# francescobrigante/Audio-Style-Transfer

Hardware: AMD Instinct MI355X
Metric: audio-seconds/sec/node (train step, 4s@22.05kHz pairs) (higher is better)
Workload: dtype bf16; 1 GPU; configs[1]: batch=8 4 s clips per GPU (S=2, x=(B,S,2,287,597)), full train2 step: STFT + CQT front-end from resident waveforms, encoders+decoder+discriminator, all losses, D and G phases, grad clip, Adam; global_batch=8, parallelism=dp1, hip_graph=True, dp_semantics=per-rank BN and batch-coupled losses

## Files before the change

audio-style-transfer_amd/ast_amd/_lib.py:

```python
from __future__ import annotations

import ctypes as C
import os

import torch

_HERE = os.path.dirname(os.path.abspath(__file__))
LIB_PATH = os.environ.get("AST_HIP_LIB") or os.path.join(_HERE, "libast_hip.so")

F32, BF16 = 0, 1
MAX_TAPS = 9

vp, i32, i64, f32 = C.c_void_p, C.c_int32, C.c_int64, C.c_float


class Gather(C.Structure):
    _fields_ = [(n, i32) for n in ("N", "Hs", "Ws", "Cs", "Hm", "Wm", "sh", "sw", "oh", "ow", "Hd", "Wd", "Cd",
                                   "dsh", "dsw", "doh", "dow", "ntaps", "wtaps")] + [("tap", i32 * MAX_TAPS)]


class WeightDesc(C.Structure):
    _fields_ = [("w", vp), ("u", vp), ("v", vp), ("sigma", vp), ("scratch", vp), ("wf", vp), ("wb", vp)] + \
               [(n, i32) for n in ("Co", "Ci", "KK", "s_co", "s_ci", "Cop", "Cip", "power_iter")] + \
               [("dwp", vp), ("grad", vp), ("inner", vp), ("dwp_from_wb", i32), ("dwp_replicas", i32)]


class LinWg(C.Structure):
    _fields_ = [("dy", vp), ("x", vp), ("dW", vp), ("db", vp)] + [(n, i32) for n in ("M", "N", "K", "lddy", "ldw", "p0", "p1", "p2")]


_SIGS = {
    "ast_version": ([], i32),
    "ast_igemm": ([vp, vp, vp, vp, C.POINTER(Gather), i32, i32, vp, C.c_long, vp], i32),
    "ast_igemm_plan": ([C.POINTER(Gather), i32, C.POINTER(i32 * 5)], i32),
    "ast_pconv_variant": ([C.POINTER(Gather), i32, C.POINTER(i32 * 4)], i32),
    "ast_igemm_ws_floats": ([C.POINTER(Gather), i32], C.c_long),
    "ast_wgrad": ([vp, vp, vp, C.POINTER(Gather), i32, vp], i32),
    "ast_skinny_gemm": ([vp, vp, vp, vp, i32, i32, i32, i32, i32, i32, vp], i32),
    "ast_skinny_gemm_ex": ([vp, vp, vp, vp, i32, i32, i32, i32, i32, i32, vp, vp, f32, C.c_uint64, vp, vp], i32),
    "ast_bigk_gemm": ([vp, vp, vp, vp, i32, i32, i32, i32, vp], i32),
    "ast_bign_dgrad": ([vp, vp, vp, i32, i32, i32, i32, vp], i32),
    "ast_linear_wgrad": ([vp, vp, vp, vp, i32, i32, i32, i32, i32, vp], i32),
    "ast_linear_wgrad_batched": ([vp, i32, i32, vp], i32),
    "ast_linear_wgrad_batched_host": ([vp, i32, i32, vp], i32),
    "ast_nchw_to_nhwc": ([vp, vp, i32, i32, i32, i32, i64, i64, i64, i32, i32, vp], i32),
    "ast_nhwc_to_nchw": ([vp, vp, i32, i32, i32, i32, i32, i32, vp], i32),
    "ast_cast": ([vp, i32, vp, i32, i64, vp], i32),
    "ast_weights_prepare_t": ([vp, vp, i32, i32, i32, vp, i32, vp], i32),
    "ast_sn_scratch_floats": ([i32, i32], C.c_long),
    "ast_weight_grads_flush_t": ([vp, vp, i32, vp], i32),
    "ast_dropout_fwd": ([vp, vp, vp, i64, f32, C.c_uint64, vp, vp], i32),
    "ast_weight_grad_unpack": ([vp, i32, vp, vp, vp, vp, vp, i32, i32, i32, i32, i32, i32, i32, vp, vp], i32),
    "ast_chan_stats": ([vp, vp, i32, i32, i32, i32, i32, vp], i32),
    "ast_norm_finalize": ([vp, i32, vp, i32, i32, i32, i32, i32, vp, vp, vp, vp, i32, f32, vp, vp, vp, vp, C.c_long, vp], i32),
    "ast_affine_act": ([vp, vp, vp, vp, vp, vp, vp, i32, i32, i32, i32, i32, vp], i32),
    "ast_bn_apply_fwd": ([vp, vp, vp, vp, i32, C.c_long, vp, vp, vp, vp, vp, vp, f32, vp, vp, f32, vp, vp, i32, i32, i32, i32, i32, i32, vp], i32),
    "ast_bn_apply_bwd": ([vp, vp, vp, vp, vp, vp, i32, C.c_long, vp, vp, vp, vp, vp, vp, vp, vp, vp, vp, vp, vp, vp, vp, i32, i32, i32, i32, i32, i32, vp], i32),
    "ast_norm_bwd_sums": ([vp, vp, vp, vp, vp, i32, i32, i32, i32, i32, i32, vp], i32),
    "ast_norm_bwd_sums_pre": ([vp, vp, vp, vp, vp, i32, i32, i32, i32, i32, i32, vp, vp, vp, vp, vp], i32),
    "ast_norm_bwd_apply_pre": ([vp, vp, vp, vp, vp, vp, vp, vp, i32, i32, i32, i32, i32, vp, vp, vp, vp, vp], i32),
    "ast_norm_bwd_finalize": ([vp, i32, i32, i32, i32, i32, vp, vp, vp, vp, vp, vp, vp, vp, vp, vp, vp, vp, vp], i32),
    "ast_norm_bwd_finalize_n": ([vp, i32, i32, i32, i32, i32, vp, vp, vp, vp, vp, vp, vp, vp, vp, vp, vp, vp, C.c_long, vp], i32),
    "ast_igemm_bn": ([vp, vp, vp, vp, C.POINTER(Gather), i32, i32, vp, C.c_long, vp, vp, vp, vp], i32),
    "ast_norm_bwd_apply": ([vp, vp, vp, vp, vp, vp, vp, vp, i32, i32, i32, i32, i32, vp], i32),
    "ast_layernorm_fwd": ([vp, vp, vp, vp, vp, vp, i32, i32, f32, i32, vp], i32),
    "ast_layernorm_bwd": ([vp, vp, vp, vp, vp, vp, vp, vp, i32, i32, i32, vp], i32),
    "ast_add_drop_ln_fwd": ([vp, vp, vp, vp, vp, vp, vp, vp, vp, i32, i32, f32, f32, C.c_uint64, vp, vp], i32),
    "ast_add_drop_ln_bwd": ([vp, vp, vp, vp, vp, vp, vp, vp, vp, vp, vp, i32, i32, vp], i32),
    "ast_adaptive_pool_fwd": ([vp, vp, i32, i32, i32, i32, i32, i32, i32, vp], i32),
    "ast_adaptive_pool_bwd": ([vp, vp, i32, i32, i32, i32, i32, i32, i32, vp], i32),
    "ast_bilinear_fwd": ([vp, vp, i32, i32, i32, i32, i32, i32, i32, i32, vp], i32),
    "ast_bilinear_bwd": ([vp, vp, i32, i32, i32, i32, i32, i32, i32, i32, vp], i32),
    "ast_attn_fwd": ([vp, vp, vp, vp, vp, i32, i32, i32, i32, i32, i32, i32, i32, i32, vp, vp], i32),
    "ast_attn_bwd": ([vp, vp, vp, vp, vp, vp, vp, vp, i32, i32, i32, i32, i32, i32, i32, i32, vp, vp], i32),
    "ast_rowmix": ([vp, vp, vp, i32, i32, i32, vp], i32),
    "ast_attn_fwd_p": ([vp, vp, vp, vp, vp, i32, i32, i32, i32, i32, i32, i32, i32, i32, vp, f32, C.c_uint64, vp, vp], i32),
    "ast_attn_bwd_p": ([vp, vp, vp, vp, vp, vp, vp, vp, i32, i32, i32, i32, i32, i32, i32, i32, vp, f32, C.c_uint64, vp, vp], i32),
    "ast_add": ([vp, vp, vp, i64, i32, vp], i32),
    "ast_relu_bwd": ([vp, vp, vp, i64, i32, vp], i32),
    "ast_dropout_mask": ([vp, i64, f32, C.c_uint64, vp, vp], i32),
    "ast_mul": ([vp, vp, vp, i64, i32, vp], i32),
    "ast_recon_loss": ([vp, vp, i64, i32, i32, i32, i32, f32, f32, f32, f32, f32, vp, vp, vp], i32),
    "ast_recon_loss_total": ([vp, vp, i64, i32, i32, i32, i32, C.POINTER(f32), C.POINTER(f32), vp, vp, vp, vp], i32),
    "ast_infonce": ([vp, vp, i32, i32, f32, vp, vp, vp, vp], i32),
    "ast_margin": ([vp, i32, i32, f32, vp, vp, vp], i32),
    "ast_hsic": ([vp, vp, i32, i32, vp, vp, vp, vp, vp], i32),
    "ast_crosscov": ([vp, vp, i32, i32, vp, vp, vp, vp, vp], i32),
    "ast_istft": ([vp, i32, i32, vp, vp, vp], i32),
    "ast_bin_stats_acc": ([vp, vp, vp, i32, i32, i32, vp], i32),
    "ast_zscore": ([vp, vp, vp, vp, i32, i32, i32, f32, vp], i32),
    "ast_sections_overlap_avg": ([vp, vp, i32, i32, i32, i32, i32, i32, i32, vp], i32),
    "ast_cross_entropy": ([vp, vp, i32, i32, vp, vp, vp], i32),
    "ast_softmax_entropy": ([vp, i32, i32, vp, vp, vp], i32),
    "ast_scale": ([vp, vp, f32, vp, i64, i32, vp], i32),
    "ast_colsum_acc": ([vp, i64, i32, i32, vp, i32, vp], i32),
    "ast_sumsq": ([vp, i64, vp, vp], i32),
    "ast_adam": ([vp, vp, vp, vp, i64, f32, f32, f32, f32, f32, vp, vp, f32, vp], i32),
    "ast_adam_dev": ([vp, vp, vp, vp, i64, vp, f32, f32, f32, f32, vp, vp, vp], i32),
    "ast_set_values": ([vp, C.POINTER(f32), i32, vp], i32),
    "ast_weighted_sum": ([C.POINTER(vp), C.POINTER(i32), i32, vp, vp, vp], i32),
    "ast_weighted_sum_bwd": ([vp, C.POINTER(i32), i32, vp, vp, vp], i32),
    "ast_counter_incr": ([vp, vp], i32),
    "ast_stft_sections": ([vp, i32, i32, vp, vp, vp, i32, i32, i32, i32, vp], i32),
    "ast_cqt_octaves": ([vp, vp, vp, vp, vp, vp, i32, i32, vp, vp, vp, i32, vp, i32, i32, i32, vp], i32),
    "ast_cqt_sections": ([vp, i32, i32, i32, vp, vp, vp, i32, i32, i32, i32, i32, vp], i32),
    "ast_resample_poly": ([vp, i32, i32, vp, i32, i32, i32, i32, vp, i32, f32, vp], i32),
    "ast_wgrad_rep": ([vp, vp, vp, C.POINTER(Gather), i32, i32, vp], i32),
    "ast_wgrad_slab": ([vp, vp, vp, C.POINTER(Gather), i32, i32, C.POINTER(i32), vp], i32),
    "ast_slab_sum": ([C.POINTER(vp), C.POINTER(i64), C.POINTER(i32), i32, vp], i32),
    "ast_ordered_sum": ([vp, i64, i32, i32, vp, i32, vp], i32),
    "ast_igemm_ws_floats_det": ([C.POINTER(Gather), i32], C.c_long),
    "ast_sumsq_det": ([vp, i64, vp, vp, i32, vp], i32),
    "ast_colsum_acc_det": ([vp, i64, i32, i32, vp, i32, vp, i32, vp], i32),
    "ast_chan_stats_det": ([vp, vp, i32, i32, i32, i32, vp, i32, vp], i32),
    "ast_norm_bwd_sums_det": ([vp, vp, vp, vp, vp, i32, i32, i32, i32, i32, vp, vp, vp, vp, vp, i32, vp], i32),
    "ast_layernorm_bwd_det": ([vp, vp, vp, vp, vp, vp, vp, vp, i32, i32, i32, vp, vp], i32),
    "ast_add_drop_ln_bwd_det": ([vp, vp, vp, vp, vp, vp, vp, vp, vp, vp, vp, i32, i32, vp, vp], i32),
    "ast_recon_loss_total_det": ([vp, vp, i64, i32, i32, i32, i32, C.POINTER(f32), C.POINTER(f32), vp, C.c_long, vp, vp, vp], i32),
    "ast_weight_grads_flush_det": ([vp, vp, i32, vp, C.c_long, vp], i32),
    "ast_bigk_gemm_det_ws_floats": ([i32, i32, i32], C.c_long),
    "ast_bigk_gemm_det": ([vp, vp, vp, vp, i32, i32, i32, vp, C.c_long, vp], i32),
    "ast_bign_dgrad_det_ws_floats": ([i32, i32, i32], C.c_long),
    "ast_bign_dgrad_det": ([vp, vp, vp, i32, i32, i32, i32, vp, C.c_long, vp], i32),
    "ast_skinny_gemm_wide": ([vp, vp, vp, vp, i32, i32, i32, i32, i32, i32, vp], i32),
    "ast_skinny_gemm_wide_ex": ([vp, vp, vp, vp, i32, i32, i32, i32, i32, i32, vp, vp, f32, C.c_uint64, vp, vp], i32),
    "ast_linear_wgrad_wide": ([vp, vp, vp, vp, i32, i32, i32, i32, i32, vp], i32),
    "ast_bigk_gemm_wide": ([vp, vp, vp, vp, i32, i32, i32, i32, vp], i32),
    "ast_bigk_gemm_wide_det_ws_floats": ([i32, i32, i32], C.c_long),
    "ast_bigk_gemm_wide_det": ([vp, vp, vp, vp, i32, i32, i32, vp, C.c_long, vp], i32),
    "ast_bign_dgrad_wide": ([vp, vp, vp, i32, i32, i32, i32, vp], i32),
    "ast_bign_dgrad_wide_det_ws_floats": ([i32, i32, i32], C.c_long),
    "ast_bign_dgrad_wide_det": ([vp, vp, vp, i32, i32, i32, i32, vp, C.c_long, vp], i32),
    "ast_tok_max_ops": ([], i32),
    "ast_tok_program": ([vp, i32, i32, i32, vp, vp, vp, vp], i32),
}

EXPORTS = tuple(_SIGS) + ("ast_last_error",)

_lib = None


PROFILE_CALLS = None
NEXT_BYTES = None


def _es(dtype_code):
    return 2 if dtype_code == BF16 else 4


CALL_BYTES = {
    "ast_affine_act": lambda a: a[7] * a[8] * a[9] * _es(a[11]) * (2 + (1 if a[3] else 0)),
    "ast_norm_bwd_apply_pre": lambda a: a[8] * a[9] * a[10] * _es(a[12]) * (3 + (2 if a[3] else 0)),
    "ast_norm_bwd_sums_pre": lambda a: a[5] * a[6] * a[7] * _es(a[9]) * (2 + (1 if a[3] else 0)),
    "ast_bn_apply_fwd": lambda a: a[18] * a[19] * a[20] * _es(a[23]) * (2 + (1 if a[1] else 0)),
    "ast_bn_apply_bwd": lambda a: a[22] * a[23] * a[24] * _es(a[27]) * (3 + (2 if a[2] else 0)),
    "ast_chan_stats": lambda a: a[2] * a[3] * a[4] * _es(a[5]),
    "ast_recon_loss": lambda a: 3 * 4 * a[3] * a[4] * 2 * a[5] * a[6],
    "ast_recon_loss_total": lambda a: 3 * 4 * a[3] * a[4] * 2 * a[5] * a[6],
    "ast_adam": lambda a: 7 * 4 * a[4],
    "ast_sumsq": lambda a: 4 * a[1],
    "ast_weights_prepare_t": None,
    "ast_weight_grads_flush_t": None,
    "ast_nchw_to_nhwc": lambda a: a[2] * a[4] * a[5] * (a[3] * 4 + a[9] * _es(a[10])),
    "ast_bilinear_fwd": lambda a: a[0] and a[2] * (a[5] * a[6] * a[4] * _es(a[9]) + a[3] * a[7] * a[8] * 4),
}


class _ProfiledLib:
    def __init__(self, raw):
        self._raw = raw

    def __getattr__(self, name):
        fn = getattr(self._raw, name)
        if name not in CALL_BYTES:
            return fn

        def wrapped(*args):
            global NEXT_BYTES
            f = CALL_BYTES[name]
            nbytes = NEXT_BYTES if f is None else f(args)
            NEXT_BYTES = None
            e0, e1 = torch.cuda.Event(enable_timing=True), torch.cuda.Event(enable_timing=True)
            e0.record()
            rc = fn(*args)
            e1.record()
            PROFILE_CALLS.append((name, float(nbytes or 0), e0, e1))
            return rc
        return wrapped


def lib():
    global _lib
# ... 40 lines not shown
```

audio-style-transfer_amd/ast_amd/config.py:

```python
import torch

compute_dtype = torch.float32


def set_compute_dtype(dtype):
    global compute_dtype
    if dtype not in (torch.float32, torch.bfloat16):
        raise ValueError("compute dtype must be torch.float32 or torch.bfloat16")
    compute_dtype = dtype


import os as _os
fused_tokens = _os.environ.get("AST_FUSED_TOKENS", "1") != "0"
tok_programs = int(_os.environ.get("AST_TOK_PROGRAMS", "0"))

fused_bn_stats = _os.environ.get("AST_FUSED_BN_STATS", "1") != "0"

bn_mask_from_preact = _os.environ.get("AST_BN_MASK_FROM_PREACT", "1") != "0"

fused_bn_bwd = _os.environ.get("AST_FUSED_BN_BWD", "1") != "0"

wgrad_replicas = int(_os.environ.get("AST_WGRAD_REPLICAS", "8"))

fused_finalize = _os.environ.get("AST_FUSED_FINALIZE", "0") != "0"

wgrad_slabs = int(_os.environ.get("AST_WGRAD_SLABS", "0"))

wgrad_defer = _os.environ.get("AST_WGRAD_DEFER", "1") != "0"
wgrad_defer_streams = int(_os.environ.get("AST_WGRAD_DEFER_STREAMS", "1"))
wgrad_defer_pool = _os.environ.get("AST_WGRAD_DEFER_POOL", "0") != "0"
wgrad_defer_lend = float(_os.environ.get("AST_WGRAD_DEFER_LEND", "1.0"))

deterministic = _os.environ.get("AST_DETERMINISTIC", "0") not in ("", "0")


def check_deterministic_supported(flag, world=1):
    if not flag:
        return
    if tok_programs != 0:
        raise ValueError("deterministic mode: the token programs (AST_TOK_PROGRAMS != 0) add floats with atomics; set AST_TOK_PROGRAMS=0")
    if world > 1:
        raise ValueError("deterministic mode covers one GPU (world == 1); data parallelism is not supported")


def set_deterministic(flag):
    global deterministic
    flag = bool(flag)
    check_deterministic_supported(flag)
    deterministic = flag
```

audio-style-transfer_amd/ast_amd/content_encoder.py:

```python
from __future__ import annotations

import torch
import torch.nn as nn

from . import layers as L
from . import config, ops, tokprog
from .style_encoder import (CHANNELS, ResBlock, SinusoidalPositionalEncoding, _module_bank, build_resnet,
                            initialize_weights, run_resnet)


class ContentEncoder(nn.Module):

    def __init__(self, in_channels: int = 2, cnn_out_dim: int = 256, transformer_dim: int = 256, num_heads: int = 4,
                 num_layers: int = 4, channels_list: list = list(CHANNELS)):
        super().__init__()
        self.cnn, last = build_resnet(in_channels, list(channels_list))
        self.proj = nn.Linear(last, cnn_out_dim)
        self.input_proj = nn.Linear(cnn_out_dim, transformer_dim) if cnn_out_dim != transformer_dim else None
        self.pos_encoder = SinusoidalPositionalEncoding(transformer_dim)
        self.norm = nn.LayerNorm(transformer_dim)
        layer = nn.TransformerEncoderLayer(d_model=transformer_dim, nhead=num_heads, dim_feedforward=transformer_dim * 4,
                                           dropout=0.1, batch_first=True)
        self.transformer = nn.TransformerEncoder(layer, num_layers=num_layers)

    def register(self, bank):
        for m in self.cnn:
            if isinstance(m, ResBlock):
                m.register(bank)
        self._proj = bank.add(self.proj.weight, "linear", L.tok_dtype, bias=self.proj.bias)
        self._inp = bank.add(self.input_proj.weight, "linear", L.tok_dtype, bias=self.input_proj.bias) if self.input_proj else None
        self._layers = [L.EncoderLayer(bank, l) for l in self.transformer.layers]

    def forward(self, x: torch.Tensor) -> torch.Tensor:
        B, S, C, T, F = x.shape
        bank = _module_bank(self)
        bank.prepare(self.training)
        feat = run_resnet(self.cnn, ops.cached_nhwc(x, L.img_dtype()), self.training)
        feat = L.linear(feat, self._proj)
        if self._inp is not None:
            feat = L.linear(feat, self._inp)
        seq = L.layer_norm(self.pos_encoder(feat.view(B, S, -1)), self.norm)
        if config.tok_programs > 0 and tokprog.encoder_stack_ok(seq, self._layers):
            seq = tokprog.encoder_stack(seq, self._layers, self.training, xcd=1)
        else:
            for lyr in self._layers:
                seq = lyr(seq, self.training)
        return seq
```

audio-style-transfer_amd/ast_amd/layers.py:

```python
from __future__ import annotations

import contextlib
import ctypes as C
import os

import torch
import torch.nn as nn

from . import config, ops, streams
from ._lib import LinWg, WeightDesc, check, dcode, lib, ptr, stream
from .ops import PackedWeight, pad8


class WeightBank:

    def __init__(self):
        self.specs = []
        self.entries: list[PackedWeight] = []
        self._key = None
        self._keys = {}
        self._flush_pending = False
        self._flush_stream = None
        self._lin_deferred = []
        self._pinned = []
# ... 248 lines not shown
                    rounds.append([])
                rounds[r].append(rec)
            if torch.cuda.is_current_stream_capturing():
                self._pinned.append(items)
            for rr in rounds:
                arr = (LinWg * len(rr))(*rr)
                check(lib().ast_linear_wgrad_batched_host(C.addressof(arr), len(rr), max_tiles, stream()), "ast_linear_wgrad_batched_host")


class _ParallelFlush:
    active = False
    pending = []


class _DeferPool:
    banks = []
    cost = staticmethod(lambda it: float(it[3].N) * it[3].Hm * it[3].Wm * max(it[3].Cd, 32) * max(it[3].ntaps * it[3].Cs, 64))

    @staticmethod
    def _run(lane, items):
        for dy, src, dwp, g, replicas, pw in sorted(items, key=_DeferPool.cost, reverse=True):
            dy.record_stream(lane)
            src.record_stream(lane)
            with torch.cuda.stream(lane):
                ops._wgrad_launch(dy, src, dwp, g, replicas, pw)

    @staticmethod
    def launch_all(origin):
        banks, _DeferPool.banks = [b for b in _DeferPool.banks if b._conv_deferred], []
        cost = _DeferPool.cost
        tot = [sum(cost(it) for it in b._conv_deferred) for b in banks]
        h = tot.index(min(tot))
        target = sum(tot) / len(banks)
        room = max(0.0, target - tot[h]) * config.wgrad_defer_lend
        lent = []
        for bi, b in enumerate(banks):
            keep = list(b._conv_deferred)
            if bi != h and room > 0:
                give = min(tot[bi] - target, room * (tot[bi] - target) / max(1e-9, sum(max(0.0, t - target) for i, t in enumerate(tot) if i != h)))
                keep.sort(key=cost)
                while keep and give >= cost(keep[0]):
                    give -= cost(keep[0])
                    lent.append(keep.pop(0))
                if len(keep) < len(b._conv_deferred):
                    b._wait_lane = banks[h]._side_stream(origin)
            b._conv_deferred = []
            _DeferPool._run(b._side_stream(origin), keep)
        helper = banks[h]
        if lent:
            helper._flush_conv_kernels(helper._side_stream(origin))
            helper._pool_flushed = True
            _DeferPool._run(helper._side_stream(origin), lent)


@contextlib.contextmanager
def parallel_flush():
    if os.environ.get("AST_PARALLEL_FLUSH", "1") == "0":
        yield
        return
    _ParallelFlush.active, _ParallelFlush.pending = True, []
    _DeferPool.banks = []
    try:
        yield
    finally:
        _ParallelFlush.active = False
        cur = torch.cuda.current_stream()
        for s in _ParallelFlush.pending:
            streams.join(cur, s)
        _ParallelFlush.pending = []


def img_dtype():
    return config.compute_dtype


def tok_dtype():
    return torch.float32


def _link_of(x):
    return getattr(x, "_bn_link", None)


def conv(x, pw, k, stride, pad, bias_grad):
    return ops.Conv2dFn.apply(x, pw.weight, pw, k, stride, pad, bias_grad, None, _link_of(x))


def convT(x, pw, k, stride, pad, out_pad, bias_grad):
    return ops.ConvT2dFn.apply(x, pw.weight, pw, k, stride, pad, out_pad, bias_grad, None, _link_of(x))


def _bn_apply(y, bn, training, relu, stats):
    link = ops.BNLink() if (training and config.fused_bn_bwd) else None
    out = ops.BatchNormActFn.apply(y, bn.weight, bn.bias, bn, training, relu, stats, link)
    if link is not None:
        out._bn_link = link
    return out


def linear(x2d, pw, relu=False):
    y = ops.LinearFn.apply(x2d, pw.weight, pw, relu)
    return y if pw.Cop == pw.Co else y[:, :pw.Co]


def bn_act(x, bn: nn.BatchNorm2d, training, relu=True, stats=None):
    return _bn_apply(x, bn, training, relu, stats)


def conv_with_stats(x, pw, k, stride, pad, training):
    stats = None
    if training and config.fused_bn_stats:
        N, H, W, Cs = x.shape
        g, _ = ops.gather_direct(N, H, W, Cs, pw.Cop, k, stride, pad)
        if ops.stats_fusable(g, ops.dcode(x.dtype)):
            stats = ops.stat_table(ops.stat_slots(pw.Cop) * pw.Cop * 2, x.device)
    return ops.Conv2dFn.apply(x, pw.weight, pw, k, stride, pad, False, stats, _link_of(x)), stats


def convT_bn_act(x, pw, k, stride, pad, out_pad, bn: nn.BatchNorm2d, training, relu=True):
    stats = None
    if training and config.fused_bn_stats:
        N, H, W, Cs = x.shape
        Ho = (H - 1) * stride - 2 * pad + k + out_pad
        Wo = (W - 1) * stride - 2 * pad + k + out_pad
        gs = ops.gathers_transposed(N, H, W, Cs, Ho, Wo, pw.Cop, k, stride, pad)
        if all(ops.stats_fusable(g, ops.dcode(x.dtype)) for g in gs):
            stats = ops.stat_table(ops.stat_slots(pw.Cop) * pw.Cop * 2, x.device)
    y = ops.ConvT2dFn.apply(x, pw.weight, pw, k, stride, pad, out_pad, False, stats, _link_of(x))
    return _bn_apply(y, bn, training, relu, stats)


def res_head(x, p1, pd, stride, training):
    stats = None
    if training and config.fused_bn_stats:
        N, H, W, Cs = x.shape
        g, _ = ops.gather_direct(N, H, W, Cs, p1.Cop, 3, stride, 1)
        if ops.stats_fusable(g, ops.dcode(x.dtype)):
            stats = ops.stat_table(ops.stat_slots(p1.Cop) * p1.Cop * 2, x.device)
    in_stats = None
    if training and config.fused_bn_stats:
        N, H, W, Cs = x.shape
        gd, _ = ops.gather_direct(N, H, W, Cs, pd.Cop, 1, stride, 0)
        if ops.in_stats_fusable(gd, ops.dcode(x.dtype)):
            in_stats = ops.stat_table(N * pd.Cop * 2, x.device)
    c1, idn = ops.ResHeadFn.apply(x, p1.weight, pd.weight, p1, pd, stride, stats, in_stats)
    return c1, idn, stats, in_stats


def conv_bn_act(x, pw, k, stride, pad, bn: nn.BatchNorm2d, training, relu=True):
    y, stats = conv_with_stats(x, pw, k, stride, pad, training)
    return _bn_apply(y, bn, training, relu, stats)


def layer_norm(x, ln: nn.LayerNorm):
    return ops.LayerNormFn.apply(x, ln.weight, ln.bias, ln.eps)


class MHA:

    def __init__(self, bank: WeightBank, m: nn.MultiheadAttention, cross: bool):
        d = m.embed_dim
        self.m, self.d, self.h, self.cross = m, d, m.num_heads, cross
        if cross:
            self.q = bank.add(m.in_proj_weight, "linear", tok_dtype, bias=m.in_proj_bias, rows=(0, d))
            self.kv = bank.add(m.in_proj_weight, "linear", tok_dtype, bias=m.in_proj_bias, rows=(d, 3 * d))
        else:
            self.qkv = bank.add(m.in_proj_weight, "linear", tok_dtype, bias=m.in_proj_bias)
        self.out = bank.add(m.out_proj.weight, "linear", tok_dtype, bias=m.out_proj.bias)

    def __call__(self, x, mem, training, p_drop, causal=False):
        B, Lq, d = x.shape
        dh = d // self.h
        if self.cross:
            Lk = mem.shape[1]
            q = linear(x.reshape(B * Lq, d), self.q)
            kv = linear(mem.reshape(B * Lk, d), self.kv)
            k_off, v_off = 0, d
        else:
            Lk = Lq
            q = kv = linear(x.reshape(B * Lq, d), self.qkv)
            k_off, v_off = d, 2 * d
        o = ops.AttnCoreFn.apply(q, kv, B, self.h, Lq, Lk, dh, k_off, v_off, causal, float(p_drop) if training else 0.0)
        return linear(o, self.out).view(B, Lq, d)


class EncoderLayer:

    def __init__(self, bank, layer: nn.TransformerEncoderLayer):
        self.l = layer
        self.attn = MHA(bank, layer.self_attn, cross=False)
        self.ff1 = bank.add(layer.linear1.weight, "linear", tok_dtype, bias=layer.linear1.bias)
        self.ff2 = bank.add(layer.linear2.weight, "linear", tok_dtype, bias=layer.linear2.bias)

    def __call__(self, x, training):
        l, p = self.l, self.l.dropout.p
        B, L, d = x.shape
        if not config.fused_tokens:
            x = layer_norm(x + ops.dropout(self.attn(x, None, training, l.self_attn.dropout), l.dropout1.p, training), l.norm1)
            h = ops.dropout(linear(x.reshape(B * L, d), self.ff1, relu=True), p, training)
            h = ops.dropout(linear(h, self.ff2), l.dropout2.p, training).view(B, L, d)
            return layer_norm(x + h, l.norm2)
        _, x = ops.add_drop_ln(x, self.attn(x, None, training, l.self_attn.dropout), l.norm1, l.dropout1.p, training)
        h = ops.ffn(x.reshape(B * L, d), self.ff1, self.ff2, p, training)
        _, y = ops.add_drop_ln(x, h.view(B, L, d), l.norm2, l.dropout2.p, training)
        return y


class DecoderLayer:

    def __init__(self, bank, layer: nn.TransformerDecoderLayer):
        self.l = layer
        self.sa = MHA(bank, layer.self_attn, cross=False)
        self.ca = MHA(bank, layer.multihead_attn, cross=True)
        self.ff1 = bank.add(layer.linear1.weight, "linear", tok_dtype, bias=layer.linear1.bias)
        self.ff2 = bank.add(layer.linear2.weight, "linear", tok_dtype, bias=layer.linear2.bias)

    def __call__(self, x, memory, training):
        l = self.l
        B, L, d = x.shape
        if not config.fused_tokens:
            h = layer_norm(x, l.norm1)
            x = x + ops.dropout(self.sa(h, None, training, l.self_attn.dropout, causal=True), l.dropout1.p, training)
            h = layer_norm(x, l.norm2)
            x = x + ops.dropout(self.ca(h, memory, training, l.multihead_attn.dropout), l.dropout2.p, training)
            h = layer_norm(x, l.norm3)
            h = ops.dropout(linear(h.reshape(B * L, d), self.ff1, relu=True), l.dropout.p, training)
            h = ops.dropout(linear(h, self.ff2), l.dropout3.p, training).view(B, L, d)
            return x + h
        h = layer_norm(x, l.norm1)
        x, h = ops.add_drop_ln(x, self.sa(h, None, training, l.self_attn.dropout, causal=True), l.norm2, l.dropout1.p, training)
        x, h = ops.add_drop_ln(x, self.ca(h, memory, training, l.multihead_attn.dropout), l.norm3, l.dropout2.p, training)
        h = ops.ffn(h.reshape(B * L, d), self.ff1, self.ff2, l.dropout.p, training)
        x, _ = ops.add_drop_ln(x, h.view(B, L, d), None, l.dropout3.p, training)
        return x

    def memory_kv(self, memory):
        B, Lm, d = memory.shape
        return linear(memory.reshape(B * Lm, d), self.ca.kv), Lm

    def step(self, x_t, kv_self, mem_kv):
        l = self.l
        B, _, d = x_t.shape
        dh = d // self.sa.h
        h = layer_norm(x_t, l.norm1).reshape(B, d)
        qkv = linear(h, self.sa.qkv)
        new_kv = qkv[:, d:].reshape(B, 1, 2 * d)
        kv_self = new_kv if kv_self is None else torch.cat([kv_self, new_kv], dim=1)
        t1 = kv_self.shape[1]
        q = qkv[:, :d].contiguous()
        o = ops.AttnCoreFn.apply(q, kv_self.reshape(B * t1, 2 * d), B, self.sa.h, 1, t1, dh, 0, d, False, 0.0)
        x = x_t.reshape(B, d) + linear(o, self.sa.out)
        h = layer_norm(x, l.norm2)
        kvm, Lm = mem_kv
        o = ops.AttnCoreFn.apply(linear(h, self.ca.q), kvm, B, self.ca.h, 1, Lm, dh, 0, d, False, 0.0)
        x = x + linear(o, self.ca.out)
        h = layer_norm(x, l.norm3)
        x = x + linear(linear(h, self.ff1, relu=True), self.ff2)
        return x.view(B, 1, d), kv_self
```

audio-style-transfer_amd/ast_amd/new_decoder.py:

```python
from __future__ import annotations

import torch
import torch.nn as nn
from torch.nn.utils import spectral_norm

from . import layers as L
from . import config, ops, tokprog
from .style_encoder import SinusoidalPositionalEncoding, _module_bank

ENC_CH = ((2, 16, 1), (16, 32, 2), (32, 64, 2), (64, 64, 2))
DEC_CH = ((1, 64), (64, 32), (32, 16), (16, 8))


def _conv_bn_relu_slots(conv, ch):
    return [conv, nn.BatchNorm2d(ch), nn.Identity()]


class Decoder(nn.Module):

    def __init__(self, d_model=256, nhead=4, num_layers=4, dim_feedforward=1024, dropout=0.1, max_seq_len=1000):
        super().__init__()
        self.d_model, self.max_seq_len = d_model, max_seq_len
        self.F_compressed, self.T_compressed, self.feature_dim = 32, 16, 64
        enc = []
        for cin, cout, s in ENC_CH:
            enc += _conv_bn_relu_slots(spectral_norm(nn.Conv2d(cin, cout, kernel_size=3, stride=s, padding=1)), cout)
        enc.append(nn.AdaptiveAvgPool2d((self.F_compressed, self.T_compressed)))
        self.conv_encoder = nn.Sequential(*enc)
        fd = self.feature_dim
        self.spatial_projection = nn.Sequential(
            *_conv_bn_relu_slots(spectral_norm(nn.Conv2d(fd, fd, kernel_size=3, padding=1)), fd),
            spectral_norm(nn.Conv2d(fd, 1, kernel_size=1)))
        self.feature_to_sequence = nn.Linear(self.F_compressed * self.T_compressed, d_model)
        self.sequence_to_feature = nn.Linear(d_model, self.F_compressed * self.T_compressed)
        dec = []
        for cin, cout in DEC_CH:
            dec += _conv_bn_relu_slots(
                spectral_norm(nn.ConvTranspose2d(cin, cout, kernel_size=3, stride=2, padding=1, output_padding=1)), cout)
        dec.append(spectral_norm(nn.ConvTranspose2d(8, 2, kernel_size=3, padding=1)))
        dec.append(nn.Upsample(size=(287, 513), mode="bilinear", align_corners=False))
        self.conv_decoder = nn.Sequential(*dec)
        self.content_proj = nn.Linear(d_model, d_model)
        self.class_proj = nn.Linear(d_model, d_model)
        self.pos_encoding = SinusoidalPositionalEncoding(d_model)
        layer = nn.TransformerDecoderLayer(d_model=d_model, nhead=nhead, dim_feedforward=dim_feedforward, dropout=dropout,
                                           batch_first=True, norm_first=True)
        self.transformer_decoder = nn.TransformerDecoder(layer, num_layers=num_layers)
        self.start_token = nn.Parameter(torch.randn(1, 1, d_model))
        self.input_norm = nn.LayerNorm(d_model)
        self.output_norm = nn.LayerNorm(d_model)
        self.dropout = nn.Dropout(dropout)
        self._init_weights()

    def _init_weights(self):
        for name, p in self.named_parameters():
            if "weight" in name:
                nn.init.xavier_uniform_(p, gain=0.2) if p.dim() > 1 else nn.init.zeros_(p)
            elif "bias" in name:
                nn.init.zeros_(p)

    def register(self, bank):
        conv = lambda c: bank.add(c.weight_orig, "conv", L.img_dtype, u=c.weight_u, v=c.weight_v, bias=c.bias)
        convt = lambda c: bank.add(c.weight_orig, "convT", L.img_dtype, u=c.weight_u, v=c.weight_v, bias=c.bias)
        lin = lambda l: bank.add(l.weight, "linear", L.tok_dtype, bias=l.bias)
        self._enc = [conv(self.conv_encoder[i]) for i in (0, 3, 6, 9)]
        self._sp = [conv(self.spatial_projection[0]), conv(self.spatial_projection[3])]
        self._dec = [convt(self.conv_decoder[i]) for i in (0, 3, 6, 9, 12)]
        self._f2s, self._s2f = lin(self.feature_to_sequence), lin(self.sequence_to_feature)
        self._cp, self._kp = lin(self.content_proj), lin(self.class_proj)
        self._layers = [L.DecoderLayer(bank, l) for l in self.transformer_decoder.layers]

    def _prepare(self):
        _module_bank(self).prepare(self.training)

    def _encode_nhwc(self, h):
        tr = self.training
        for pw, i, (_, _, s) in zip(self._enc, (0, 3, 6, 9), ENC_CH):
            h = L.conv_bn_act(h, pw, 3, s, 1, self.conv_encoder[i + 1], tr, relu=True)
        h = ops.AdaptivePoolFn.apply(h, self.F_compressed, self.T_compressed)
        h = L.conv_bn_act(h, self._sp[0], 3, 1, 1, self.spatial_projection[1], tr, relu=True)
        h = L.conv(h, self._sp[1], 1, 1, 0, True)
        flat = ops.CastFn.apply(h[..., 0].reshape(h.shape[0], -1), torch.float32)
        return L.linear(flat, self._f2s)

    def encode_input(self, x):
        self._prepare()
        return self._encode_nhwc(ops.nchw_to_nhwc(x, L.img_dtype()))

    def _generate(self, tok):
        B, S, D = tok.shape
        tr = self.training
        h = L.linear(L.layer_norm(tok, self.output_norm).reshape(B * S, D), self._s2f)
        h = ops.CastFn.apply(h, L.img_dtype()).view(B * S, self.F_compressed, self.T_compressed, 1)
        h = torch.cat([h, h.new_zeros(B * S, self.F_compressed, self.T_compressed, 7)], dim=3)
        for pw, i in zip(self._dec[:4], (0, 3, 6, 9)):
            h = L.convT_bn_act(h, pw, 3, 2, 1, 1, self.conv_decoder[i + 1], tr, relu=True)
        h = L.convT(h, self._dec[4], 3, 1, 1, 0, True)
        out = ops.BilinearToNCHWFn.apply(h, 2, 287, 513)
        return out.view(B, S, 2, 287, 513)

    def generate_output(self, decoder_outputs):
        self._prepare()
        return self._generate(decoder_outputs)

    def create_causal_mask(self, seq_len):
        return torch.triu(torch.ones(seq_len, seq_len), diagonal=1).bool()

    def _memory(self, content_emb, class_emb):
        B, Sc, D = content_emb.shape
        if 2 * Sc > ops.ATTN_MAX_L:
            raise ValueError(f"{Sc} content sections make {2 * Sc} memory tokens; the attention core takes {ops.ATTN_MAX_L} "
                             f"(at most {ops.ATTN_MAX_L // 2} sections per clip)")
        cm = L.linear(content_emb.reshape(B * Sc, D), self._cp).view(B, Sc, D)
        km = L.linear(class_emb, self._kp).unsqueeze(1).expand(-1, Sc, -1)
        return ops.dropout(torch.cat([cm, km], dim=1), self.dropout.p, self.training)

    def prepare_memory(self, content_emb, class_emb):
        self._prepare()
        return self._memory(content_emb, class_emb)

    def _stack(self, tgt, memory):
        if config.tok_programs > 0 and tokprog.decoder_stack_ok(tgt, memory, self._layers):
            return tokprog.decoder_stack(tgt, memory, self._layers, self.training)
        for lyr in self._layers:
            tgt = lyr(tgt, memory, self.training)
        return tgt

    def encode_target(self, y):
        self._prepare()
        B, S = y.shape[:2]
        return self._encode_nhwc(ops.nchw_to_nhwc(y.view(B * S, *y.shape[2:]), L.img_dtype())).view(B, S, self.d_model)

    def _training_pass(self, y, memory, y_embeddings=None):
        B, S = y.shape[:2]
        emb = y_embeddings
        if emb is None:
            emb = self._encode_nhwc(ops.nchw_to_nhwc(y.view(B * S, *y.shape[2:]), L.img_dtype())).view(B, S, self.d_model)
        tgt = torch.cat([self.start_token.expand(B, 1, -1), emb[:, :-1, :]], dim=1)
        tgt = L.layer_norm(self.pos_encoding(tgt), self.input_norm)
        return self._generate(self._stack(tgt, memory))

    def forward_training(self, y, memory):
        self._prepare()
        return self._training_pass(y, memory)

    decode_mode = "recompute"

    def _inference_pass_cached(self, memory, target_length):
        B, d = memory.size(0), self.d_model
        mem_kv = [lyr.memory_kv(memory) for lyr in self._layers]
        caches = [None] * len(self._layers)
        tok = self.start_token.expand(B, -1, -1)
        pe = self.pos_encoding.pe
        outs = []
        for t in range(target_length):
            x = tok + pe[:, t:t + 1]
            for i, lyr in enumerate(self._layers):
                x, caches[i] = lyr.step(x, caches[i], mem_kv[i])
            outs.append(x)
            tok = x
        return self._generate(torch.cat(outs, dim=1))

    def _inference_pass(self, memory, target_length=None):
        B = memory.size(0)
        if target_length is None:
            target_length = memory.size(1) // 2
        if target_length > self.pos_encoding.pe.size(1):
            raise ValueError(f"target_length {target_length}, but the positional table holds {self.pos_encoding.pe.size(1)} positions")
        if self.decode_mode == "kv_cache" and not torch.is_grad_enabled():
            return self._inference_pass_cached(memory, target_length)
        seq = self.start_token.expand(B, -1, -1)
        outs = []
        for _ in range(target_length):
            nxt = self._stack(self.pos_encoding(seq), memory)[:, -1:, :]
            outs.append(nxt)
            seq = torch.cat([seq, nxt], dim=1)
        return self._generate(torch.cat(outs, dim=1))

    def forward_inference(self, memory, target_length=None):
        self._prepare()
        return self._inference_pass(memory, target_length)

    def forward(self, content_emb, class_emb, y=None, target_length=None, y_embeddings=None):
        if y_embeddings is None or not (self.training and y is not None):
            self._prepare()
        memory = self._memory(content_emb, class_emb)
        if self.training and y is not None:
            if len(y.shape) != 5:
                raise ValueError(f"Expected y to have shape [B, S, 2, 287, 513], got {y.shape}")
            return self._training_pass(y, memory, y_embeddings)
        return self._inference_pass(memory, target_length)


def compute_comprehensive_loss(output, target, lambda_temporal=0.3, lambda_phase=0.2, lambda_spectral=0.1):
    return _comprehensive_loss(output, target, lambda_temporal, lambda_phase, lambda_spectral, 2.0)


def _comprehensive_loss(output, target, lambda_temporal, lambda_phase, lambda_spectral, mse_weight):
    B, S, _, Freq, T = output.shape
    n = B * S * Freq * T
    c = (mse_weight / (2 * n), 0.5 / n, lambda_phase / n,
         (lambda_temporal / (2 * B * (S - 1) * Freq * T)) if S > 1 else 0.0,
         (lambda_spectral / (2 * B * S * (Freq - 1) * T)) if Freq > 1 else 0.0)
    inv = (1.0 / (2 * n), 1.0 / n, 1.0 / n,
           1.0 / (2 * B * (S - 1) * Freq * T) if S > 1 else 0.0,
           1.0 / (2 * B * S * (Freq - 1) * T) if Freq > 1 else 0.0)
    total, _, parts = ops.ReconTotalFn.apply(output.contiguous(), target, c, inv)
    return {"total_loss": total, "mse_loss": parts[0], "mag_loss": parts[1], "phase_loss": parts[2],
            "temporal_loss": parts[3], "spectral_loss": parts[4]}
```

audio-style-transfer_amd/ast_amd/ops.py:

```python
from __future__ import annotations

import ctypes
import functools
import math

import torch

from . import _lib, config
from ._lib import Gather, check, dcode, lib, ptr, stream


@functools.lru_cache(maxsize=None)
def const_tensor(values, dtype, device):
    return torch.tensor(values, dtype=dtype, device=device)


def pad8(c: int) -> int:
    return (c + 7) // 8 * 8


def _tap(dh, dw, wt):
    return (dh + 64) | ((dw + 64) << 8) | (wt << 16)


# ... 254 lines not shown

class Conv2dFn(torch.autograd.Function):

    @staticmethod
    def forward(ctx, x, weight, pw: PackedWeight, k, stride, pad, bias_grad, stats=None, link=None):
        N, H, W, Cs = x.shape
        g, (Ho, Wo) = gather_direct(N, H, W, Cs, pw.Cop, k, stride, pad)
        y = torch.empty((N, Ho, Wo, pw.Cop), dtype=x.dtype, device=x.device)
        _igemm(x, pw.wf, pw.bias_ptr_tensor(), y, g, stats=stats)
        ctx.save_for_backward(x)
        ctx.pw, ctx.geom, ctx.args, ctx.bias_grad, ctx.link = pw, g, (k, stride, pad), bias_grad, link
        return y

    @staticmethod
    def backward(ctx, dy):
        (x,) = ctx.saved_tensors
        pw, (k, stride, pad) = ctx.pw, ctx.args
        dy = dy.contiguous()
        N, H, W, Cs = x.shape
        if pw.dwp is None:
            raise RuntimeError("weights were prepared in eval/no-grad mode; run the forward in training mode before backward")
        _wgrad(dy, x, pw.dwp, ctx.geom, pw.replicas, pw)
        pw.bank.request_flush()
        if ctx.bias_grad:
            pw.add_bias_grad(dy)
        dx = None
        if ctx.needs_input_grad[0]:
            dx = torch.empty_like(x)
            gs = gathers_transposed(N, dy.shape[1], dy.shape[2], pw.Cop, H, W, Cs, k, stride, pad)
            link = _bn_link_ready(ctx.link, gs, x)
            for g in gs:
                _igemm(dy, pw.wb, None, dx, g, bn=link)
            if link is not None:
                link.filled = True
        return dx, None, None, None, None, None, None, None, None


def _bn_link_ready(link, geoms, x):
    if link is None or link.x is None or not config.fused_bn_bwd or _SyncBN.active:
        return None
    if not all(stats_fusable(g, dcode(x.dtype)) for g in geoms):
        return None
    link.slots = stat_slots(x.shape[3])
    link.table = stat_table(link.slots * x.shape[3] * 3, x.device)
    return link



class ResHeadFn(torch.autograd.Function):

    @staticmethod
    def forward(ctx, x, w1, wd, pw1: PackedWeight, pwd: PackedWeight, stride, stats, in_stats=None):
        N, H, W, Cs = x.shape
        g1, (Ho, Wo) = gather_direct(N, H, W, Cs, pw1.Cop, 3, stride, 1)
        gd, (Hd, Wd) = gather_direct(N, H, W, Cs, pwd.Cop, 1, stride, 0)
        assert (Ho, Wo) == (Hd, Wd)
        c1 = torch.empty((N, Ho, Wo, pw1.Cop), dtype=x.dtype, device=x.device)
        idn = torch.empty((N, Ho, Wo, pwd.Cop), dtype=x.dtype, device=x.device)
        _igemm(x, pw1.wf, pw1.bias_ptr_tensor(), c1, g1, stats=stats)
        _igemm(x, pwd.wf, pwd.bias_ptr_tensor(), idn, gd, stats=in_stats, per_image=in_stats is not None)
        ctx.save_for_backward(x)
        ctx.pws, ctx.geoms, ctx.stride = (pw1, pwd), (g1, gd), stride
        return c1, idn

    @staticmethod
    def backward(ctx, dc1, didn):
        (x,) = ctx.saved_tensors
        (pw1, pwd), (g1, gd), stride = ctx.pws, ctx.geoms, ctx.stride
        dc1, didn = dc1.contiguous(), didn.contiguous()
        N, H, W, Cs = x.shape
        if pw1.dwp is None or pwd.dwp is None:
            raise RuntimeError("weights were prepared in eval/no-grad mode; run the forward in training mode before backward")
        _wgrad(dc1, x, pw1.dwp, g1, pw1.replicas, pw1)
        _wgrad(didn, x, pwd.dwp, gd, pwd.replicas, pwd)
        pw1.bank.request_flush()
        dx = None
        if ctx.needs_input_grad[0]:
            dx = torch.empty_like(x)
            Ho, Wo = dc1.shape[1], dc1.shape[2]
            for g in gathers_transposed(N, Ho, Wo, pw1.Cop, H, W, Cs, 3, stride, 1):
                _igemm(dc1, pw1.wb, None, dx, g)
            for g in gathers_transposed(N, Ho, Wo, pwd.Cop, H, W, Cs, 1, stride, 0):
                if g.ntaps > 0:
                    _igemm(didn, pwd.wb, None, dx, g, flags=1)
        return dx, None, None, None, None, None, None, None


class ConvT2dFn(torch.autograd.Function):

    @staticmethod
    def forward(ctx, x, weight, pw: PackedWeight, k, stride, pad, out_pad, bias_grad, stats=None, link=None):
        N, H, W, Cs = x.shape
        Ho = (H - 1) * stride - 2 * pad + k + out_pad
        Wo = (W - 1) * stride - 2 * pad + k + out_pad
        y = torch.empty((N, Ho, Wo, pw.Cop), dtype=x.dtype, device=x.device)
        b = pw.bias_ptr_tensor()
        for g in gathers_transposed(N, H, W, Cs, Ho, Wo, pw.Cop, k, stride, pad):
            _igemm(x, pw.wf, b, y, g, stats=stats)
        ctx.save_for_backward(x)
        ctx.pw, ctx.args, ctx.bias_grad, ctx.link = pw, (k, stride, pad, Ho, Wo), bias_grad, link
        return y

    @staticmethod
    def backward(ctx, dy):
        (x,) = ctx.saved_tensors
        pw, (k, stride, pad, Ho, Wo) = ctx.pw, ctx.args
        dy = dy.contiguous()
        N, H, W, Cs = x.shape
        g, (Hx, Wx) = gather_direct(N, Ho, Wo, pw.Cop, Cs, k, stride, pad)
        assert (Hx, Wx) == (H, W), "ConvTranspose2d geometry mismatch"
        if pw.dwp is None:
            raise RuntimeError("weights were prepared in eval/no-grad mode; run the forward in training mode before backward")
        _wgrad(x, dy, pw.dwp, g, pw.replicas, pw)
        pw.bank.request_flush()
        if ctx.bias_grad:
            pw.add_bias_grad(dy)
        dx = None
        if ctx.needs_input_grad[0]:
            dx = torch.empty_like(x)
            link = _bn_link_ready(ctx.link, (g,), x)
            _igemm(dy, pw.wb, None, dx, g, bn=link)
            if link is not None:
                link.filled = True
        return dx, None, None, None, None, None, None, None, None, None


SKINNY_MAX_ROWS = 64
WIDE_MAX_ROWS = 1024
ATTN_MAX_L = 1024


def _skinny_gemm(rows, *args):
    x, w, b, y, *rest = args
    name = "ast_skinny_gemm" if rows <= SKINNY_MAX_ROWS else "ast_skinny_gemm_wide"
    check(getattr(lib(), name)(x, w, b, y, rows, *rest, stream()), name)


def _skinny_gemm_ex(rows, *args):
    x, w, b, y, *rest = args
    name = "ast_skinny_gemm_ex" if rows <= SKINNY_MAX_ROWS else "ast_skinny_gemm_wide_ex"
    check(getattr(lib(), name)(x, w, b, y, rows, *rest, stream()), name)


def _linear_wgrad(rows, *args):
    dy, x, dw, db, *rest = args
    name = "ast_linear_wgrad" if rows <= SKINNY_MAX_ROWS else "ast_linear_wgrad_wide"
    check(getattr(lib(), name)(dy, x, dw, db, rows, *rest, stream()), name)


def _token_rows_ok(rows):
    return rows <= SKINNY_MAX_ROWS or (config.deterministic and rows <= WIDE_MAX_ROWS)


class LinearFn(torch.autograd.Function):

    @staticmethod
    def forward(ctx, x, weight, pw: PackedWeight, relu):
        x = x.contiguous()
        rows = x.shape[0]
        assert x.shape[1] == pw.Cip and x.dtype == pw.dtype, (x.shape, pw.Cip, x.dtype, pw.dtype)
        ctx.skinny = (_token_rows_ok(rows) and pw.KK == 1 and pw.u is None and pw.Ci == pw.Cip
                      and (rows <= SKINNY_MAX_ROWS or x.dtype == torch.float32))
        y = torch.empty((rows, pw.Cop), dtype=x.dtype, device=x.device)
        if ctx.skinny:
            if pw.Cop != pw.Co:
                y.zero_()
            b = None if pw.bias is None else pw.bias.data_ptr() + 4 * pw.b_off
            _skinny_gemm(rows, ptr(x), pw.weight.data_ptr() + 4 * pw.w_off, b, ptr(y), pw.Co, pw.Ci, pw.s_co, pw.Cop, int(relu))
        else:
            g, _ = gather_direct(rows, 1, 1, pw.Cip, pw.Cop, 1, 1, 0)
            _igemm(x, pw.wf, pw.bias_ptr_tensor(), y, g, 2 if relu else 0)
        ctx.save_for_backward(x, y if relu else None)
        ctx.pw, ctx.relu = pw, relu
        return y

    @staticmethod
    def backward(ctx, dy):
        x, y = ctx.saved_tensors
        pw = ctx.pw
        dy = dy.contiguous()
        rows = x.shape[0]
        if ctx.relu:
            dz = torch.empty_like(dy)
            check(lib().ast_relu_bwd(ptr(dy), ptr(y), ptr(dz), dy.numel(), dcode(dy.dtype), stream()), "ast_relu_bwd")
            dy = dz
        dx = None
        if ctx.skinny:
            if pw.bank is not None:
                pw.bank.defer_linear_wgrad(pw, dy, x)
            else:
                gw = acc_grad(pw.weight)
                gb = None if pw.bias is None else acc_grad(pw.bias).data_ptr() + 4 * pw.b_off
                _linear_wgrad(rows, ptr(dy), ptr(x), gw.data_ptr() + 4 * pw.w_off, gb, pw.Co, pw.Ci, pw.Cop, pw.s_co)
            if ctx.needs_input_grad[0]:
                dx = torch.empty_like(x)
                _skinny_gemm(rows, ptr(dy), ptr(pw.wb), None, ptr(dx), pw.Ci, pw.Cop, pw.Cop, pw.Cip, 0)
            return dx, None, None, None
        if config.deterministic:
            raise RuntimeError(f"LinearFn: the non-skinny weight gradient (> {WIDE_MAX_ROWS} token rows, spectral norm, unpadded channels "
                               "or bf16 above 64 rows) has no deterministic form")
        g, _ = gather_direct(rows, 1, 1, pw.Cip, pw.Cop, 1, 1, 0)
        dwp = torch.zeros((pw.Cop, 1, pw.Cip), dtype=torch.float32, device=x.device)
        _wgrad(dy, x, dwp, g)
        pw.add_weight_grad(dwp, 0)
        pw.add_bias_grad(dy)
        if ctx.needs_input_grad[0]:
            gb, _ = gather_direct(rows, 1, 1, pw.Cop, pw.Cip, 1, 1, 0)
            dx = torch.empty_like(x)
            _igemm(dy, pw.wb, None, dx, gb)
        return dx, None, None, None


class BigLinearFn(torch.autograd.Function):

    @staticmethod
    def forward(ctx, x, weight, bias):
        x = x.contiguous()
        rows, K = x.shape
        N = weight.shape[0]
        assert weight.shape[1] == K and x.dtype == torch.float32 and weight.is_contiguous()
        if rows > WIDE_MAX_ROWS:
            raise RuntimeError(f"BigLinearFn: {rows} token rows > {WIDE_MAX_ROWS} (the cap of the wide token path, AST_WIDE_MAX_ROWS)")
        y = torch.empty((rows, N), dtype=torch.float32, device=x.device)
        ctx.big_in = K > N
        sfx = "" if rows <= SKINNY_MAX_ROWS else "_wide"
        if ctx.big_in and config.deterministic:
            ws = det_ws(getattr(lib(), f"ast_bigk_gemm{sfx}_det_ws_floats")(rows, N, K), x.device)
            check(getattr(lib(), f"ast_bigk_gemm{sfx}_det")(ptr(x), ptr(weight), ptr(bias), ptr(y), rows, N, K, ptr(ws), ws.numel(), stream()),
                  f"ast_bigk_gemm{sfx}_det")
        elif ctx.big_in:
            check(getattr(lib(), f"ast_bigk_gemm{sfx}")(ptr(x), ptr(weight), ptr(bias), ptr(y), rows, N, K, N, stream()), f"ast_bigk_gemm{sfx}")
        else:
            _skinny_gemm(rows, ptr(x), ptr(weight), ptr(bias), ptr(y), N, K, K, N, 0)
        ctx.save_for_backward(x)
        ctx.weight, ctx.bias = weight, bias
        return y

    @staticmethod
    def backward(ctx, dy):
        (x,) = ctx.saved_tensors
        w, b = ctx.weight, ctx.bias
        dy = dy.contiguous()
        rows, K = x.shape
        N = w.shape[0]
        _linear_wgrad(rows, ptr(dy), ptr(x), ptr(acc_grad(w)), ptr(acc_grad(b)) if b is not None else None, N, K, N, K)
        dx = None
        if ctx.needs_input_grad[0]:
            if ctx.big_in:
                raise NotImplementedError("BigLinearFn: input gradient of the huge-input linear (its input is data on the reference's path)")
            dx = torch.empty_like(x)
            sfx = "" if rows <= SKINNY_MAX_ROWS else "_wide"
            if config.deterministic:
                ws = det_ws(getattr(lib(), f"ast_bign_dgrad{sfx}_det_ws_floats")(rows, N, K), x.device)
                check(getattr(lib(), f"ast_bign_dgrad{sfx}_det")(ptr(dy), ptr(w), ptr(dx), rows, N, K, N, ptr(ws), ws.numel(), stream()),
                      f"ast_bign_dgrad{sfx}_det")
            else:
                check(getattr(lib(), f"ast_bign_dgrad{sfx}")(ptr(dy), ptr(w), ptr(dx), rows, N, K, N, stream()), f"ast_bign_dgrad{sfx}")
        return dx, None, None


class FFNFn(torch.autograd.Function):

    @staticmethod
    def forward(ctx, x, w1, w2, pw1: PackedWeight, pw2: PackedWeight, p):
        x = x.contiguous()
        rows = x.shape[0]
        h = torch.empty((rows, pw1.Cop), dtype=x.dtype, device=x.device)
        y = torch.empty((rows, pw2.Cop), dtype=x.dtype, device=x.device)
        mask, seed, ctr = None, 0, None
        if p > 0.0:
            if _DropState.counter is None or _DropState.counter.device != x.device:
                _DropState.counter = torch.zeros(1, dtype=torch.int64, device=x.device)
            _DropState.calls += 1
            seed, ctr = _DropState.seed + 7919 * _DropState.calls, _DropState.counter
            mask = torch.empty_like(h)
        _skinny_gemm_ex(rows, ptr(x), pw1.weight.data_ptr() + 4 * pw1.w_off, pw1.bias.data_ptr() + 4 * pw1.b_off, ptr(h),
                        pw1.Co, pw1.Ci, pw1.s_co, pw1.Cop, 1, None, ptr(mask), float(p), seed, ptr(ctr))
        _skinny_gemm(rows, ptr(h), pw2.weight.data_ptr() + 4 * pw2.w_off, pw2.bias.data_ptr() + 4 * pw2.b_off, ptr(y),
                     pw2.Co, pw2.Ci, pw2.s_co, pw2.Cop, 0)
        ctx.save_for_backward(x, h, mask)
        ctx.pw1, ctx.pw2 = pw1, pw2
        return y

    @staticmethod
    def backward(ctx, dy):
        x, h, mask = ctx.saved_tensors
        pw1, pw2 = ctx.pw1, ctx.pw2
        dy = dy.contiguous()
        rows = x.shape[0]
        pw2.bank.defer_linear_wgrad(pw2, dy, h)
        dh = torch.empty_like(h)
        if mask is None:
            _skinny_gemm(rows, ptr(dy), ptr(pw2.wb), None, ptr(dh), pw2.Ci, pw2.Cop, pw2.Cop, pw2.Cip, 0)
            dz = torch.empty_like(dh)
            check(lib().ast_relu_bwd(ptr(dh), ptr(h), ptr(dz), dh.numel(), dcode(dh.dtype), stream()), "ast_relu_bwd")
            dh = dz
        else:
            _skinny_gemm_ex(rows, ptr(dy), ptr(pw2.wb), None, ptr(dh), pw2.Ci, pw2.Cop, pw2.Cop, pw2.Cip, 0, ptr(mask), None, 0.0, 0, None)
        pw1.bank.defer_linear_wgrad(pw1, dh, x)
        dx = None
        if ctx.needs_input_grad[0]:
            dx = torch.empty_like(x)
            _skinny_gemm(rows, ptr(dh), ptr(pw1.wb), None, ptr(dx), pw1.Ci, pw1.Cop, pw1.Cop, pw1.Cip, 0)
        return dx, None, None, None, None, None


def _skinny_ok(pw, rows):
    return (_token_rows_ok(rows) and pw.KK == 1 and pw.u is None and pw.Ci == pw.Cip and pw.Co == pw.Cop and pw.bank is not None
            and pw.bias is not None)


def ffn(x2d, pw1, pw2, p, training):
    rows = x2d.shape[0]
    if _skinny_ok(pw1, rows) and _skinny_ok(pw2, rows) and x2d.dtype == torch.float32:
        return FFNFn.apply(x2d, pw1.weight, pw2.weight, pw1, pw2, float(p) if training else 0.0)
    h = dropout(LinearFn.apply(x2d, pw1.weight, pw1, True), p, training)
    h = h if pw1.Cop == pw1.Co else h[:, :pw1.Co]
    y = LinearFn.apply(h, pw2.weight, pw2, False)
    return y if pw2.Cop == pw2.Co else y[:, :pw2.Co]


_scratch = {}


def _clean_scratch(n, device, tag=None):
    key = (n, device, torch.cuda.current_stream(device).cuda_stream, tag)
    t = _scratch.get(key)
    if t is None:
        t = _scratch[key] = torch.zeros(n, dtype=torch.float32, device=device)
    return t


def det_slots(rows, per=1):
    return max(1, min(512 // per, (int(rows) + 255) // 256))


def det_ws(n, device):
    return _clean_scratch(max(1, int(n)), device, tag="det")


def _stats(x):
    N, H, W, C = x.shape
    sums = stat_table(N * C * 2, x.device)
    if config.deterministic:
        ns = det_slots(H * W, N)
        check(lib().ast_chan_stats_det(ptr(x), ptr(sums), N, H * W, C, dcode(x.dtype), ptr(det_ws(N * ns * C * 2, x.device)), ns, stream()),
              "ast_chan_stats_det")
        return sums
    check(lib().ast_chan_stats(ptr(x), ptr(sums), N, H * W, C, dcode(x.dtype), 1, stream()), "ast_chan_stats")
    return sums


def _bwd_sums(dy, y, x, r, sums3, N, HW, C, relu, dt, scale1, shift1, scale2, shift2):
    y, r, scale1, shift1, scale2, shift2 = (t if (t is None or isinstance(t, int)) else ptr(t) for t in (y, r, scale1, shift1, scale2, shift2))
    if config.deterministic:
        ns = det_slots(HW, N)
        check(lib().ast_norm_bwd_sums_det(ptr(dy), y, ptr(x), r, ptr(sums3), N, HW, C, int(relu), dt, scale1, shift1,
                                          scale2, shift2, ptr(det_ws(N * ns * C * 3, dy.device)), ns, stream()), "ast_norm_bwd_sums_det")
        return
    check(lib().ast_norm_bwd_sums_pre(ptr(dy), y, ptr(x), r, ptr(sums3), N, HW, C, int(relu), dt, 1,
                                      scale1, shift1, scale2, shift2, stream()), "ast_norm_bwd_sums")


class _SyncBN:
    world = 1
    group = None
    active = False


def set_sync_bn(world=1, group=None, force=False):
    _SyncBN.world, _SyncBN.group = int(world), group
    _SyncBN.active = _SyncBN.world > 1 or bool(force)


def _global_sums(sums, n_floats):
    import torch.distributed as dist
    g = sums[:n_floats].clone()
    dist.all_reduce(g, op=dist.ReduceOp.SUM, group=_SyncBN.group)
    return g


def _bn_batch_stats(x, gamma, beta, bn, stats=None):
    N, H, W, C = x.shape
    rows = stats.numel() // (2 * C) if stats is not None else N
    sums = stats if stats is not None else _stats(x)
    pixels = N * H * W
    if _SyncBN.active:
        g = _global_sums(sums, rows * C * 2)
        sums[:rows * C * 2].zero_()
        out = torch.empty((4, C), dtype=torch.float32, device=x.device)
        check(lib().ast_norm_finalize(ptr(g), 0, ptr(bn.num_batches_tracked), rows, 0, C, gamma.numel(), 0, ptr(gamma),
                                      ptr(beta), ptr(bn.running_mean), ptr(bn.running_var), 0, bn.eps, ptr(out[0]), ptr(out[1]),
                                      ptr(out[2]), ptr(out[3]), pixels * _SyncBN.world, stream()), "ast_norm_finalize")
        return out[0], out[1], out[2], out[3]
    return _finalize(sums, rows, H * W, C, gamma.numel(), False, gamma, beta, bn.running_mean, bn.running_var, False, bn.eps, x.device,
                     nbt=bn.num_batches_tracked, count=pixels)


def _finalize(sums, N, HW, C, Creal, instance, gamma, beta, rm, rv, eval_mode, eps, dev, nbt=None, count=0):
    n = N * C if instance else C
    out = torch.empty((4, n), dtype=torch.float32, device=dev)
    mean, rstd, scale, shift = out[0], out[1], out[2], out[3]
    check(lib().ast_norm_finalize(ptr(sums), 1, ptr(nbt), N, HW, C, Creal, int(instance), ptr(gamma), ptr(beta), ptr(rm), ptr(rv),
                                  int(eval_mode), eps, ptr(mean), ptr(rstd), ptr(scale), ptr(shift), count, stream()),
          "ast_norm_finalize")
    return mean, rstd, scale, shift


class BatchNormActFn(torch.autograd.Function):

    @staticmethod
    def forward(ctx, x, gamma, beta, bn, training, relu, stats=None, link=None):
        N, H, W, C = x.shape
        Creal = gamma.numel()
        ctx.link = None
        ctx.fused = bool(training and config.fused_finalize and not _SyncBN.active)
        if ctx.fused:
            tab = stats if stats is not None else _stats(x)
            rows = tab.numel() // (2 * C)
            out = torch.empty((4, C), dtype=torch.float32, device=x.device)
            y = torch.empty_like(x)
            check(lib().ast_bn_apply_fwd(ptr(x), None, ptr(y), ptr(tab), rows, N * H * W, None, ptr(gamma), ptr(beta), ptr(bn.running_mean),
                                         ptr(bn.running_var), ptr(bn.num_batches_tracked), bn.eps, None, None, 0.0, ptr(out), None, N, H * W, C,
                                         Creal, int(relu), dcode(x.dtype), stream()), "ast_bn_apply_fwd")
            mean, rstd, scale, shift = out[0], out[1], out[2], out[3]
            if link is not None:
                link.x, link.scale, link.shift, link.relu = x, scale, shift, bool(relu)
                ctx.link = link
            ctx.save_for_backward(x, None, mean, rstd, scale, shift)
            ctx.gamma, ctx.beta, ctx.relu, ctx.training = gamma, beta, relu, training
            return y
        if training:
            mean, rstd, scale, shift = _bn_batch_stats(x, gamma, beta, bn, stats)
            if link is not None:
                link.x, link.scale, link.shift, link.relu = x, scale, shift, bool(relu)
                ctx.link = link
        else:
            mean, rstd, scale, shift = _finalize(None, N, H * W, C, Creal, False, gamma, beta, bn.running_mean,
                                                 bn.running_var, True, bn.eps, x.device)
        y = torch.empty_like(x)
        check(lib().ast_affine_act(ptr(x), ptr(scale), ptr(shift), None, None, None, ptr(y), N, H * W, C, int(relu),
                                   dcode(x.dtype), stream()), "ast_affine_act")
        ctx.save_for_backward(x, y, mean, rstd, scale, shift)
        ctx.gamma, ctx.beta, ctx.relu, ctx.training = gamma, beta, relu, training
        return y

    @staticmethod
    def backward(ctx, dy):
        x, y, mean, rstd, scale, shift = ctx.saved_tensors
        pre = config.bn_mask_from_preact and ctx.relu
        if not ctx.training:
            raise RuntimeError("BatchNormActFn: backward in eval mode is not on the reference's path")
        dy = dy.contiguous()
        N, H, W, C = x.shape
        gamma, beta = ctx.gamma, ctx.beta
        link = ctx.link
        if ctx.fused:
            if link is not None and link.filled:
                link.filled = False
                tab3, rows = link.table, link.slots
            else:
                tab3, rows = stat_table(N * C * 3, x.device), N
                _bwd_sums(dy, None, x, None, tab3, N, H * W, C, ctx.relu, dcode(x.dtype), scale, shift, None, None)
            dx = torch.empty_like(x)
            check(lib().ast_bn_apply_bwd(ptr(dy), ptr(x), None, ptr(dx), None, ptr(tab3), rows, N * H * W, ptr(gamma), ptr(mean), ptr(rstd),
                                         ptr(acc_grad(gamma)), ptr(acc_grad(beta)), None, None, None, None, None, ptr(scale), ptr(shift), None, None,
                                         N, H * W, C, gamma.numel(), int(ctx.relu), dcode(x.dtype), stream()), "ast_bn_apply_bwd")
            return dx, None, None, None, None, None, None, None
        k1 = torch.empty((C, 3), dtype=torch.float32, device=x.device)
        if link is not None and link.filled:
            link.filled = False
            check(lib().ast_norm_bwd_finalize_n(ptr(link.table), 1, link.slots, 0, C, gamma.numel(), ptr(gamma), ptr(mean), ptr(rstd),
                                                ptr(acc_grad(gamma)), ptr(acc_grad(beta)), ptr(k1), None, None, None, None, None, None,
                                                N * H * W, stream()), "ast_norm_bwd_finalize")
            gsum = None
        else:
            sums3 = _clean_scratch(N * C * 3, x.device)
            _bwd_sums(dy, y, x, None, sums3, N, H * W, C, ctx.relu, dcode(x.dtype), scale if pre else None, shift if pre else None,
                      None, None)
            gsum = _global_sums(sums3, N * C * 3) if _SyncBN.active else None
            check(lib().ast_norm_bwd_finalize(ptr(sums3), 1, N, H * W, C, gamma.numel(), ptr(gamma), ptr(mean), ptr(rstd),
                                              ptr(acc_grad(gamma)), ptr(acc_grad(beta)), ptr(k1),
                                              None, None, None, None, None, None, stream()), "ast_norm_bwd_finalize")
        if gsum is not None:
            check(lib().ast_norm_bwd_finalize(ptr(gsum), 0, N, H * W * _SyncBN.world, C, gamma.numel(), ptr(gamma), ptr(mean), ptr(rstd),
                                              None, None, ptr(k1), None, None, None, None, None, None, stream()), "ast_norm_bwd_finalize")
        dx = torch.empty_like(x)
        check(lib().ast_norm_bwd_apply_pre(ptr(dy), ptr(y), ptr(x), None, ptr(k1), None, ptr(dx), None, N, H * W, C,
                                           int(ctx.relu), dcode(x.dtype), ptr(scale) if pre else None, ptr(shift) if pre else None,
                                           None, None, stream()), "ast_norm_bwd_apply")
        return dx, None, None, None, None, None, None, None


class ResTailFn(torch.autograd.Function):

    @staticmethod
    def forward(ctx, c2, ds, g1, b1, g2, b2, bn, inn, training, stats=None, in_stats=None):
        N, H, W, C = c2.shape
        Creal = g1.numel()
        ctx.fused = bool(training and config.fused_finalize and not _SyncBN.active)
        if ctx.fused:
            tab1 = stats if stats is not None else _stats(c2)
            tab2 = in_stats if in_stats is not None else _stats(ds)
            rows1 = tab1.numel() // (2 * C)
            out1 = torch.empty((4, C), dtype=torch.float32, device=c2.device)
            out2 = torch.empty((4, N * C), dtype=torch.float32, device=c2.device)
            y = torch.empty_like(c2)
            check(lib().ast_bn_apply_fwd(ptr(c2), ptr(ds), ptr(y), ptr(tab1), rows1, N * H * W, ptr(tab2), ptr(g1), ptr(b1), ptr(bn.running_mean),
                                         ptr(bn.running_var), ptr(bn.num_batches_tracked), bn.eps, ptr(g2), ptr(b2), inn.eps, ptr(out1), ptr(out2),
                                         N, H * W, C, Creal, 1, dcode(c2.dtype), stream()), "ast_bn_apply_fwd")
            ctx.save_for_backward(c2, ds, None, out1[0], out1[1], out2[0], out2[1], out1[2], out1[3], out2[2], out2[3])
            ctx.params, ctx.training = (g1, b1, g2, b2), training
            return y
        if training:
            m1, r1, s1, f1 = _bn_batch_stats(c2, g1, b1, bn, stats)
        else:
            m1, r1, s1, f1 = _finalize(None, N, H * W, C, Creal, False, g1, b1, bn.running_mean, bn.running_var,
                                       True, bn.eps, c2.device)
        m2, r2, s2, f2 = _finalize(in_stats if in_stats is not None else _stats(ds), N, H * W, C, Creal, True, g2, b2, None, None, False,
                                   inn.eps, c2.device)
        y = torch.empty_like(c2)
        check(lib().ast_affine_act(ptr(c2), ptr(s1), ptr(f1), ptr(ds), ptr(s2), ptr(f2), ptr(y), N, H * W, C, 1,
                                   dcode(c2.dtype), stream()), "ast_affine_act")
        ctx.save_for_backward(c2, ds, y, m1, r1, m2, r2, s1, f1, s2, f2)
        ctx.params, ctx.training = (g1, b1, g2, b2), training
        return y

    @staticmethod
    def backward(ctx, dy):
        c2, ds, y, m1, r1, m2, r2, s1, f1, s2, f2 = ctx.saved_tensors
        pre = config.bn_mask_from_preact
        if not ctx.training:
            raise RuntimeError("ResTailFn: backward in eval mode is not on the reference's path")
        g1, b1, g2, b2 = ctx.params
        dy = dy.contiguous()
        N, H, W, C = c2.shape
        dev = c2.device
        if ctx.fused:
            tab3 = stat_table(N * C * 3, dev)
            _bwd_sums(dy, None, c2, ds, tab3, N, H * W, C, 1, dcode(c2.dtype), s1, f1, s2, f2)
            dc2, dds = torch.empty_like(c2), torch.empty_like(ds)
            check(lib().ast_bn_apply_bwd(ptr(dy), ptr(c2), ptr(ds), ptr(dc2), ptr(dds), ptr(tab3), N, N * H * W, ptr(g1), ptr(m1), ptr(r1),
                                         ptr(acc_grad(g1)), ptr(acc_grad(b1)), ptr(g2), ptr(m2), ptr(r2), ptr(acc_grad(g2)), ptr(acc_grad(b2)),
                                         ptr(s1), ptr(f1), ptr(s2), ptr(f2), N, H * W, C, g1.numel(), 1, dcode(c2.dtype), stream()), "ast_bn_apply_bwd")
            return dc2, dds, None, None, None, None, None, None, None, None, None
        sums3 = _clean_scratch(N * C * 3, dev)
        coef = (ptr(s1), ptr(f1), ptr(s2), ptr(f2)) if pre else (None, None, None, None)
        _bwd_sums(dy, y, c2, ds, sums3, N, H * W, C, 1, dcode(c2.dtype), *coef)
        k1 = torch.empty((C, 3), dtype=torch.float32, device=dev)
        k2 = torch.empty((N, C, 3), dtype=torch.float32, device=dev)
        gsum = _global_sums(sums3, N * C * 3) if _SyncBN.active else None
        check(lib().ast_norm_bwd_finalize(ptr(sums3), 1, N, H * W, C, g1.numel(), ptr(g1), ptr(m1), ptr(r1),
                                          ptr(acc_grad(g1)), ptr(acc_grad(b1)), ptr(k1), ptr(g2), ptr(m2), ptr(r2),
                                          ptr(acc_grad(g2)), ptr(acc_grad(b2)), ptr(k2), stream()),
              "ast_norm_bwd_finalize")
        if gsum is not None:
            check(lib().ast_norm_bwd_finalize(ptr(gsum), 0, N, H * W * _SyncBN.world, C, g1.numel(), ptr(g1), ptr(m1), ptr(r1),
                                              None, None, ptr(k1), None, None, None, None, None, None, stream()), "ast_norm_bwd_finalize")
        dc2, dds = torch.empty_like(c2), torch.empty_like(ds)
        check(lib().ast_norm_bwd_apply_pre(ptr(dy), ptr(y), ptr(c2), ptr(ds), ptr(k1), ptr(k2), ptr(dc2), ptr(dds), N, H * W,
                                           C, 1, dcode(c2.dtype), *coef, stream()), "ast_norm_bwd_apply")
        return dc2, dds, None, None, None, None, None, None, None, None, None


class LayerNormFn(torch.autograd.Function):
    @staticmethod
    def forward(ctx, x, gamma, beta, eps):
        shape = x.shape
        x2 = x.contiguous().view(-1, shape[-1])
        rows, D = x2.shape
        y = torch.empty_like(x2)
        mean = torch.empty(rows, dtype=torch.float32, device=x.device)
        rstd = torch.empty_like(mean)
        check(lib().ast_layernorm_fwd(ptr(x2), ptr(gamma), ptr(beta), ptr(y), ptr(mean), ptr(rstd), rows, D, eps,
                                      dcode(x2.dtype), stream()), "ast_layernorm_fwd")
        ctx.save_for_backward(x2, mean, rstd)
        ctx.gamma, ctx.beta, ctx.shape = gamma, beta, shape
        return y.view(shape)

    @staticmethod
    def backward(ctx, dy):
        x2, mean, rstd = ctx.saved_tensors
        rows, D = x2.shape
        dy2 = dy.contiguous().view(rows, D)
        dx = torch.empty_like(x2)
        if config.deterministic:
            check(lib().ast_layernorm_bwd_det(ptr(dy2), ptr(x2), ptr(ctx.gamma), ptr(mean), ptr(rstd), ptr(dx), ptr(acc_grad(ctx.gamma)),
                                              ptr(acc_grad(ctx.beta)), rows, D, dcode(x2.dtype), ptr(det_ws(2 * rows * D, dx.device)),
                                              stream()), "ast_layernorm_bwd_det")
            return dx.view(ctx.shape), None, None, None
        check(lib().ast_layernorm_bwd(ptr(dy2), ptr(x2), ptr(ctx.gamma), ptr(mean), ptr(rstd), ptr(dx),
                                      ptr(acc_grad(ctx.gamma)), ptr(acc_grad(ctx.beta)), rows, D, dcode(x2.dtype),
                                      stream()), "ast_layernorm_bwd")
        return dx.view(ctx.shape), None, None, None


class AddDropLNFn(torch.autograd.Function):

    @staticmethod
    def forward(ctx, x, sub, ln, p):
        ctx.set_materialize_grads(False)
        shape = sub.shape
        D = shape[-1]
        sub2 = sub.contiguous().view(-1, D)
        x2 = x.contiguous().view(-1, D) if x is not None else None
        rows = sub2.shape[0]
        s = torch.empty_like(sub2)
        mask = torch.empty_like(sub2) if p > 0.0 else None
        seed = 0
        if p > 0.0:
            if _DropState.counter is None or _DropState.counter.device != sub.device:
                _DropState.counter = torch.zeros(1, dtype=torch.int64, device=sub.device)
            _DropState.calls += 1
            seed = _DropState.seed + 7919 * _DropState.calls
        y = mean = rstd = None
        if ln is not None:
            y = torch.empty_like(sub2)
            mean = torch.empty(rows, dtype=torch.float32, device=sub.device)
            rstd = torch.empty_like(mean)
        check(lib().ast_add_drop_ln_fwd(ptr(x2), ptr(sub2), ptr(mask), ptr(s), ptr(ln.weight) if ln is not None else None,
                                        ptr(ln.bias) if ln is not None else None, ptr(y), ptr(mean), ptr(rstd), rows, D,
                                        float(ln.eps) if ln is not None else 0.0, float(p), seed,
                                        ptr(_DropState.counter) if p > 0.0 else None, stream()), "ast_add_drop_ln_fwd")
        ctx.save_for_backward(s, mean, rstd, mask)
        ctx.ln, ctx.shape, ctx.has_x = ln, shape, x is not None
        if ln is None:
            return s.view(shape)
        return s.view(shape), y.view(shape)

    @staticmethod
    def backward(ctx, ds_ext, dy=None):
        s, mean, rstd, mask = ctx.saved_tensors
        rows, D = s.shape
        if ds_ext is None and dy is None:
            return None, None, None, None
        ds2 = ds_ext.contiguous().view(rows, D) if ds_ext is not None else None
        dy2 = dy.contiguous().view(rows, D) if dy is not None else None
        want_dx = ctx.has_x and ctx.needs_input_grad[0]
        dx = None if (not want_dx or dy2 is None) else torch.empty_like(s)
        if dy2 is None and mask is None:
            return (ds_ext if want_dx else None), ds_ext, None, None
        dsub = torch.empty_like(s)
        ln = ctx.ln
        if config.deterministic:
            check(lib().ast_add_drop_ln_bwd_det(ptr(dy2), ptr(ds2), ptr(s), ptr(ln.weight) if dy2 is not None else None, ptr(mean),
                                                ptr(rstd), ptr(mask), ptr(dx), ptr(dsub),
                                                ptr(acc_grad(ln.weight)) if dy2 is not None else None,
                                                ptr(acc_grad(ln.bias)) if dy2 is not None else None, rows, D,
                                                ptr(det_ws(2 * rows * D, dsub.device)), stream()), "ast_add_drop_ln_bwd_det")
        else:
            check(lib().ast_add_drop_ln_bwd(ptr(dy2), ptr(ds2), ptr(s), ptr(ln.weight) if dy2 is not None else None, ptr(mean), ptr(rstd),
                                            ptr(mask), ptr(dx), ptr(dsub), ptr(acc_grad(ln.weight)) if dy2 is not None else None,
                                            ptr(acc_grad(ln.bias)) if dy2 is not None else None, rows, D, stream()), "ast_add_drop_ln_bwd")
        if want_dx and dx is None:
            dx = ds2
        return (dx.view(ctx.shape) if want_dx else None), dsub.view(ctx.shape), None, None


def add_drop_ln(x, sub, ln, p, training):
    out = AddDropLNFn.apply(x, sub, ln, float(p) if training else 0.0)
    return (out, None) if ln is None else out


class RowMixFn(torch.autograd.Function):

    @staticmethod
    def forward(ctx, x, A, At):
        x = x.contiguous()
        R_out, R_in = A.shape
        assert x.shape[0] == R_in and x.dtype == torch.float32
        y = torch.empty((R_out, x.shape[1]), dtype=torch.float32, device=x.device)
        check(lib().ast_rowmix(ptr(A), ptr(x), ptr(y), R_out, R_in, x.shape[1], stream()), "ast_rowmix")
        ctx.At = At
        return y

    @staticmethod
    def backward(ctx, dy):
        At = ctx.At
        dy = dy.contiguous()
        dx = torch.empty((At.shape[0], dy.shape[1]), dtype=torch.float32, device=dy.device)
        check(lib().ast_rowmix(ptr(At), ptr(dy), ptr(dx), At.shape[0], At.shape[1], dy.shape[1], stream()), "ast_rowmix")
        return dx, None, None


@functools.lru_cache(maxsize=256)
def _mix_matrices(kind, key, device):
    if kind == "proto":
        classes = sorted(set(key))
        A = torch.zeros(len(classes), len(key))
        for r, cid in enumerate(classes):
            idx = [i for i, v in enumerate(key) if v == cid]
            A[r, idx] = 1.0 / len(idx)
    elif kind == "gather":
        classes = sorted(set(key))
        A = torch.zeros(len(key), len(classes))
        for b, v in enumerate(key):
            A[b, classes.index(v)] = 1.0
    else:
        B, S = key
        A = torch.zeros(B, B * S)
        for b in range(B):
            A[b, b * S:(b + 1) * S] = 1.0 / S
    return A.to(device).contiguous(), A.t().contiguous().to(device)


def mul_const(x, c):
    y = torch.empty_like(x)
    check(lib().ast_mul(ptr(x.contiguous()), ptr(c), ptr(y), x.numel(), 0, stream()), "ast_mul")
    return y


def class_means(emb, labels_host):
    A, At = _mix_matrices("proto", tuple(int(v) for v in labels_host.tolist()), emb.device)
    return RowMixFn.apply(emb, A, At)


def class_rows(class_emb, labels_host):
    A, At = _mix_matrices("gather", tuple(int(v) for v in labels_host.tolist()), class_emb.device)
    return RowMixFn.apply(class_emb, A, At)


def mean_over_sections(x):
    B, S, d = x.shape
    if S == 1:
        return x.reshape(B, d)
    A, At = _mix_matrices("mean", (B, S), x.device)
    return RowMixFn.apply(x.reshape(B * S, d), A, At)


class AdaptivePoolFn(torch.autograd.Function):
    @staticmethod
    def forward(ctx, x, Ho, Wo):
        N, H, W, C = x.shape
        y = torch.empty((N, Ho, Wo, C), dtype=x.dtype, device=x.device)
        check(lib().ast_adaptive_pool_fwd(ptr(x), ptr(y), N, H, W, C, Ho, Wo, dcode(x.dtype), stream()), "pool_fwd")
        ctx.dims = (N, H, W, C, Ho, Wo)
        return y

    @staticmethod
    def backward(ctx, dy):
        N, H, W, C, Ho, Wo = ctx.dims
        dy = dy.contiguous()
        dx = torch.empty((N, H, W, C), dtype=dy.dtype, device=dy.device)
        check(lib().ast_adaptive_pool_bwd(ptr(dy), ptr(dx), N, H, W, C, Ho, Wo, dcode(dy.dtype), stream()), "pool_bwd")
        return dx, None, None


class BilinearToNCHWFn(torch.autograd.Function):

    @staticmethod
    def forward(ctx, x, C, Ho, Wo):
        N, H, W, Cp = x.shape
        y = torch.empty((N, C, Ho, Wo), dtype=torch.float32, device=x.device)
        check(lib().ast_bilinear_fwd(ptr(x), ptr(y), N, C, Cp, H, W, Ho, Wo, dcode(x.dtype), stream()), "bilinear_fwd")
        ctx.dims, ctx.dtype = (N, C, Cp, H, W, Ho, Wo), x.dtype
        return y

    @staticmethod
    def backward(ctx, dy):
        N, C, Cp, H, W, Ho, Wo = ctx.dims
        dy = dy.contiguous()
        dx = torch.empty((N, H, W, Cp), dtype=ctx.dtype, device=dy.device)
        check(lib().ast_bilinear_bwd(ptr(dy), ptr(dx), N, C, Cp, H, W, Ho, Wo, dcode(ctx.dtype), stream()), "bilinear_bwd")
        return dx, None, None, None


def nchw_to_nhwc(x4, dtype, Cp=None):
    N, Cc, H, W = x4.shape
    assert x4.dtype == torch.float32 and x4.stride(3) == 1, "expects f32 with contiguous last dim"
    Cp = Cp or pad8(Cc)
    y = torch.empty((N, H, W, Cp), dtype=dtype, device=x4.device)
    check(lib().ast_nchw_to_nhwc(ptr(x4), ptr(y), N, Cc, H, W, x4.stride(0), x4.stride(1), x4.stride(2), Cp, dcode(dtype),
                                 stream()), "ast_nchw_to_nhwc")
    return y


# ... 326 lines not shown
```

audio-style-transfer_amd/ast_amd/style_encoder.py:

```python
from __future__ import annotations

import math

import torch
import torch.nn as nn
from torch.nn.utils import spectral_norm

from . import layers as L
from . import config, ops, tokprog

CHANNELS = (32, 64, 128, 256, 512, 512)


class SinusoidalPositionalEncoding(nn.Module):

    def __init__(self, hidden_dim: int, max_len: int = 500):
        super().__init__()
        pos = torch.arange(max_len, dtype=torch.float32)[:, None]
        freq = torch.exp(torch.arange(0, hidden_dim, 2, dtype=torch.float32) * (-math.log(10000.0) / hidden_dim))
        table = torch.zeros(max_len, hidden_dim)
        table[:, 0::2], table[:, 1::2] = torch.sin(pos * freq), torch.cos(pos * freq)
        self.register_buffer("pe", table[None])

    def forward(self, x):
        if x.size(1) > self.pe.size(1):
            raise ValueError(f"{x.size(1)} tokens, but the positional table holds {self.pe.size(1)} positions")
        return x + self.pe[:, :x.size(1)]


class ResBlock(nn.Module):

    def __init__(self, in_channels: int, out_channels: int, downsample: bool = False):
        super().__init__()
        self.stride = 2 if downsample else 1
        mk = lambda ci, co, k, s, p: spectral_norm(nn.Conv2d(ci, co, k, stride=s, padding=p))
        self.conv1 = mk(in_channels, out_channels, 3, self.stride, 1)
        self.bn1 = nn.BatchNorm2d(out_channels)
        self.conv2 = mk(out_channels, out_channels, 3, 1, 1)
        self.bn2 = nn.BatchNorm2d(out_channels)
        if downsample or in_channels != out_channels:
            self.downsample = nn.Sequential(mk(in_channels, out_channels, 1, self.stride, 0),
                                            nn.InstanceNorm2d(out_channels, affine=True))
        else:
            self.downsample = nn.Identity()

    def register(self, bank: L.WeightBank):
        if isinstance(self.downsample, nn.Identity):
            raise NotImplementedError("identity shortcut: not on the reference's configured path (all 6 blocks downsample)")
        add = lambda c: bank.add(c.weight_orig, "conv", L.img_dtype, u=c.weight_u, v=c.weight_v, bias=c.bias)
        self._pw = (add(self.conv1), add(self.conv2), add(self.downsample[0]))

    def run(self, x, training):
        p1, p2, pd = self._pw
        c1, idn, c1_stats, in_stats = L.res_head(x, p1, pd, self.stride, training)
        h = L.bn_act(c1, self.bn1, training, True, c1_stats)
        c2, c2_stats = L.conv_with_stats(h, p2, 3, 1, 1, training)
        inn = self.downsample[1]
        return ops.ResTailFn.apply(c2, idn, self.bn2.weight, self.bn2.bias, inn.weight, inn.bias, self.bn2, inn, training, c2_stats, in_stats)


def build_resnet(in_channels, channels_list):
    mods, prev = [], in_channels
    for c in channels_list:
        mods.append(ResBlock(prev, c, downsample=True))
        prev = c
    mods += [nn.AdaptiveAvgPool2d((2, 5)), nn.AdaptiveAvgPool2d((1, 1))]
    return nn.Sequential(*mods), prev


def run_resnet(net: nn.Sequential, x_nhwc, training):
    h = x_nhwc
    for m in net:
        if isinstance(m, ResBlock):
            h = m.run(h, training)
        else:
            h = ops.AdaptivePoolFn.apply(h, *m.output_size)
    return ops.CastFn.apply(h.reshape(h.shape[0], -1), torch.float32)


class DeepCNN(nn.Module):

    def __init__(self, in_channels: int, out_dim: int, channels_list=CHANNELS):
        super().__init__()
        self.net, last = build_resnet(in_channels, list(channels_list))
        self.proj = nn.Linear(last, out_dim)

    def register(self, bank):
        for m in self.net:
            if isinstance(m, ResBlock):
                m.register(bank)
        self._proj = bank.add(self.proj.weight, "linear", L.tok_dtype, bias=self.proj.bias)

    def run(self, x_nhwc, training):
        return L.linear(run_resnet(self.net, x_nhwc, training), self._proj)

    def forward(self, x):
        bank = _module_bank(self)
        bank.prepare(self.training)
        return self.run(ops.nchw_to_nhwc(x, L.img_dtype()), self.training)


def _module_bank(mod):
    bank = mod.__dict__.get("_bank")
    if bank is None:
        bank = L.WeightBank()
        mod.register(bank)
        mod.__dict__["_bank"] = bank
    return bank


def class_prototypes(style_emb, labels):
    return ops.class_means(style_emb, labels)


class StyleEncoder(nn.Module):

    def __init__(self, in_channels: int = 2, cnn_out_dim: int = 256, transformer_dim: int = 256, num_heads: int = 4,
                 num_layers: int = 4, use_cls: bool = True):
        super().__init__()
        self.use_cls = use_cls
        self.cnn = DeepCNN(in_channels, cnn_out_dim)
        self.input_proj = nn.Linear(cnn_out_dim, transformer_dim) if cnn_out_dim != transformer_dim else None
        self.pos_encoder = SinusoidalPositionalEncoding(transformer_dim)
        self.norm = nn.LayerNorm(transformer_dim)
        layer = nn.TransformerEncoderLayer(d_model=transformer_dim, nhead=num_heads, dim_feedforward=transformer_dim * 4,
                                           dropout=0.1, batch_first=True)
        self.transformer = nn.TransformerEncoder(layer, num_layers=num_layers)
        if use_cls:
            self.cls_token = nn.Parameter(torch.randn(1, 1, transformer_dim))

    def register(self, bank):
        self.cnn.register(bank)
        self._inp = bank.add(self.input_proj.weight, "linear", L.tok_dtype, bias=self.input_proj.bias) if self.input_proj else None
        self._layers = [L.EncoderLayer(bank, l) for l in self.transformer.layers]

    def forward(self, x: torch.Tensor, labels: torch.Tensor = None):
        B, S, C, T, F = x.shape
        bank = _module_bank(self)
        bank.prepare(self.training)
        feat = self.cnn.run(ops.cached_nhwc(x, L.img_dtype()), self.training)
        if self._inp is not None:
            feat = L.linear(feat, self._inp)
        seq = feat.view(B, S, -1)
        if self.use_cls:
            seq = torch.cat([self.cls_token.expand(B, -1, -1), seq], dim=1)
        seq = L.layer_norm(self.pos_encoder(seq), self.norm)
        if config.tok_programs > 0 and tokprog.encoder_stack_ok(seq, self._layers):
            seq = tokprog.encoder_stack(seq, self._layers, self.training, xcd=0)
        else:
            for lyr in self._layers:
                seq = lyr(seq, self.training)
        style_emb = seq[:, 0, :] if self.use_cls else seq.mean(dim=1)
        class_emb = class_prototypes(style_emb, labels) if labels is not None else None
        return style_emb, class_emb


def initialize_weights(model):
    for _, m in model.named_modules():
        if isinstance(m, nn.Conv2d):
            nn.init.kaiming_normal_(getattr(m, "weight_orig", m.weight), mode="fan_in", nonlinearity="relu")
            if m.bias is not None:
                nn.init.zeros_(m.bias)
        elif isinstance(m, (nn.BatchNorm2d, nn.InstanceNorm2d)):
            if getattr(m, "weight", None) is not None:
                nn.init.ones_(m.weight)
            if getattr(m, "bias", None) is not None:
                nn.init.zeros_(m.bias)
        elif isinstance(m, nn.Linear):
            nn.init.xavier_normal_(m.weight, gain=0.2)
            if m.bias is not None:
                nn.init.zeros_(m.bias)
        elif isinstance(m, nn.TransformerEncoderLayer):
            for w in (m.self_attn.in_proj_weight, m.self_attn.out_proj.weight, m.linear1.weight, m.linear2.weight):
                nn.init.xavier_normal_(w, gain=0.2)
            for b in (m.self_attn.in_proj_bias, m.self_attn.out_proj.bias, m.linear1.bias, m.linear2.bias):
                nn.init.zeros_(b)
```

audio-style-transfer_amd/ast_amd/train.py:

```python
from __future__ import annotations

import dataclasses
import os

import torch
import torch.distributed as dist

from . import config, ops, streams
from ._lib import check, lib, ptr, stream
from .content_encoder import ContentEncoder
from .discriminator import Discriminator
from .losses import adversarial_loss, disentanglement_loss, infoNCE_loss, margin_loss
from .new_decoder import Decoder, compute_comprehensive_loss
from .parallel import gather_rows, global_labels
from .style_encoder import StyleEncoder, _module_bank, class_prototypes, initialize_weights
from . import layers as layers_mod


H_LR_G, H_LR_D, H_W_REC, H_W_NCE, H_W_MARGIN, H_W_HSIC, H_W_ADV = 0, 2, 4, 5, 6, 7, 8


@dataclasses.dataclass
class TrainConfig:
    lr_g: float = 1e-4
# ... 483 lines not shown
            else:
                self.G.all_reduce(self.world, self._wire_dtype, force=self._force_coll)
        if self.cfg.keep_grads:
            self.last_grad_g = self.G.flat_g.clone()
        self._seg_c(x, labels_host)
        return self._parts

    def set_frontend(self, waves, mean, std, cqt_mean=None, cqt_std=None):
        def own(slot, t):
            t = t.detach()
            key = (slot, tuple(t.shape), t.dtype, str(t.device))
            cur = self._fe_bufs.get(key)
            if cur is None:
                cur = self._fe_bufs[key] = t.contiguous().clone()
            elif cur.data_ptr() != t.data_ptr():
                cur.copy_(t)
            return cur
        self._frontend = (own("waves", waves), own("mean", mean), own("std", std))
        self._frontend_cqt = None if cqt_mean is None else (own("cqt_mean", cqt_mean), own("cqt_std", cqt_std))

    def _run_frontend(self, x):
        if self._frontend is None:
            return
        from .utilityFunctions import stft_sections
        waves, mean, std = self._frontend
        side = None
        if self._frontend_cqt is not None:
            from .cqt import cqt_sections
            if self.cfg.multi_stream and self._streams is not None and os.environ.get("AST_FRONTEND_FORK", "0") != "0":
                if self._stream_fe is None:
                    self._stream_fe = torch.cuda.Stream(device=self.device)
                main, side = torch.cuda.current_stream(), self._stream_fe
                streams.fork(side, main)
                with torch.cuda.stream(side):
                    cqt_sections(waves, x, *self._frontend_cqt)
            else:
                cqt_sections(waves, x, *self._frontend_cqt)
        stft_sections(waves, mean, std, n_sections=x.shape[1], F_total=x.shape[-1], out=x)
        if side is not None:
            streams.join(torch.cuda.current_stream(), side)

    def _deterministic(self):
        return config.deterministic if self.cfg.deterministic is None else bool(self.cfg.deterministic)

    def _check_deterministic(self):
        det = self._deterministic()
        config.check_deterministic_supported(det, self.world)

    def step(self, x: torch.Tensor, labels_host: torch.Tensor):
        self._check_deterministic()
        det = self._deterministic()
        prev, config.deterministic = config.deterministic, det
        try:
            return self._step(x, labels_host)
        finally:
            config.deterministic = prev

    def _step(self, x, labels_host):
        assert not labels_host.is_cuda, "pass labels on the host: avoids a device sync per step"
        self._sync_hyper()
        if self._dist and self._dist_in_graph is None:
            self._dist_in_graph = self._probe_collective_capture()
        if not self.cfg.use_graph or (self._matched and not self._dist_in_graph):
            self.losses = self._step_body(x, labels_host)
            return self.losses
        segmented = not self._one_graph()
        key = self._graph_key(x, labels_host, segmented)
        if key not in self._graphs:
            self._capture(key, x, labels_host, segmented)
            self._check_tok_programs(after_capture=True)
        graphs, static_x, outs = self._graphs[key]
        if static_x.data_ptr() != x.data_ptr():
            static_x.copy_(x)
        if not segmented:
            graphs[0].replay()
            if self._dist and self.world > 1 and not self._replicas_checked:
                self._check_replicas_after_first_replay()
        else:
            graphs[0].replay()
            if self._dist:
                self.D.all_reduce(self.world, force=self._force_coll)
            graphs[1].replay()
            if self._dist:
                self.G.all_reduce(self.world, self._wire_dtype, force=self._force_coll)
            graphs[2].replay()
        self.losses = outs
        self._check_tok_programs()
        return outs

    def _sync_hyper(self):
        import ctypes
        c = self.cfg
        vals = [0.0] * 9
        vals[H_LR_G], vals[H_LR_G + 1], vals[H_LR_D], vals[H_LR_D + 1] = c.lr_g, c.max_grad_norm, c.lr_d, c.max_grad_norm
        vals[H_W_REC], vals[H_W_NCE], vals[H_W_MARGIN], vals[H_W_HSIC], vals[H_W_ADV] = c.w_rec, c.w_nce, c.w_margin, c.w_hsic, c.w_adv
        vals = tuple(float(v) for v in vals)
        if vals == self._hyper_sent:
            return
        arr = (ctypes.c_float * len(vals))(*vals)
        check(lib().ast_set_values(ptr(self.hyper), arr, len(vals), stream()), "ast_set_values")
        self._hyper_sent = vals

    def _check_tok_programs(self, after_capture=False):
        if config.tok_programs != 2:
            return
        self._tok_checked = getattr(self, "_tok_checked", 0) + 1
        if not after_capture and self._tok_checked % 256:
            return
        from . import tokprog
        try:
            tokprog.check_status()
        except RuntimeError as e:
            print(f"[ast_amd] {e}; falling back to per-op token launches (AST_TOK_PROGRAMS=1)", flush=True)
            config.tok_programs = 1
            self._graphs.clear()

    def _check_replicas_after_first_replay(self):
        self._replicas_checked = True
        chk = torch.stack([self.G.flat_p.double().sum(), self.D.flat_p.double().sum()])
        lo, hi = chk.clone(), chk.clone()
        dist.all_reduce(lo, op=dist.ReduceOp.MIN)
        dist.all_reduce(hi, op=dist.ReduceOp.MAX)
        if bool(((hi - lo).abs() <= 1e-9 * (1.0 + hi.abs())).all()):
            return
        if self.rank == 0:
            print("[ast_amd] replicas diverged after a step with the collectives inside the graph: resynchronising and "
                  "falling back to the three-graph form", flush=True)
        for grp in (self.G, self.D):
            for t in (grp.flat_p, grp.m, grp.v, grp.step):
                dist.broadcast(t, src=0)
        self._dist_in_graph = False
        self._graphs.clear()

    def sync_buffers(self):
        if self.world <= 1:
            return
        for m in (self.style, self.content, self.decoder, self.disc):
            for mod in m.modules():
                if isinstance(mod, torch.nn.modules.batchnorm._BatchNorm) and mod.running_mean is not None:
                    for t in (mod.running_mean, mod.running_var):
                        dist.all_reduce(t, op=dist.ReduceOp.SUM)
                        t.div_(self.world)

    def save_checkpoint(self, path, **extra):
        from .checkpoint import save_checkpoint
        self.sync_buffers()
        if self.rank == 0:
            save_checkpoint(path, self.content, self.style, self.decoder, self.disc, **extra)

    def _graph_key(self, x, labels_host, segmented):
        c = self.cfg
        fe = tuple(t.data_ptr() for t in (self._frontend or ())) + tuple(t.data_ptr() for t in (self._frontend_cqt or ()))
        return (tuple(x.shape), tuple(labels_host.tolist()), config.compute_dtype, c.use_nce, c.use_hsic, c.use_adv, segmented,
                tuple(c.betas), c.eps, c.max_grad_norm > 0, fe, self._deterministic())

    def _mutable_state(self):
        ts = [self.G.flat_p, self.G.m, self.G.v, self.G.step, self.D.flat_p, self.D.m, self.D.v, self.D.step]
        for m in (self.style, self.content, self.decoder, self.disc):
            ts += list(m.buffers())
        if ops._DropState.counter is not None:
            ts.append(ops._DropState.counter)
        return ts

    def _capture(self, key, x, labels_host, segmented=False):
        if ops._DropState.counter is None or ops._DropState.counter.device != self.device:
            ops._DropState.counter = torch.zeros(1, dtype=torch.int64, device=self.device)
        state = self._mutable_state()
        saved = [t.clone() for t in state]
        static_x = x.clone()
        side = torch.cuda.Stream(device=self.device)
        side.wait_stream(torch.cuda.current_stream())
        with torch.cuda.stream(side):
            for _ in range(2):
                self._step_body(static_x, labels_host)
        torch.cuda.current_stream().wait_stream(side)
        torch.cuda.synchronize()
        if not segmented:
            dot = os.environ.get("AST_GRAPH_DOT")
            gph = torch.cuda.CUDAGraph(keep_graph=True) if dot else torch.cuda.CUDAGraph()
            with torch.cuda.graph(gph, **({"capture_error_mode": "thread_local"} if self._dist else {})), streams.capture_origin():
                outs = self._step_body(static_x, labels_host)
            if dot:
                import ctypes
                hip = ctypes.CDLL("libamdhip64.so")
                hip.hipGraphDebugDotPrint.argtypes = [ctypes.c_void_p, ctypes.c_char_p, ctypes.c_uint]
                rc = hip.hipGraphDebugDotPrint(ctypes.c_void_p(gph.raw_cuda_graph()), dot.encode(), 1)
                if rc != 0:
                    raise RuntimeError(f"hipGraphDebugDotPrint failed ({rc})")
                gph.instantiate()
            graphs = [gph]
        else:
            graphs = [torch.cuda.CUDAGraph() for _ in range(3)]
            pool = torch.cuda.graph_pool_handle()
            with torch.cuda.graph(graphs[0], pool=pool), streams.capture_origin():
                self._seg_a(static_x, labels_host)
            with torch.cuda.graph(graphs[1], pool=pool), streams.capture_origin():
                self._seg_b(static_x, labels_host)
            with torch.cuda.graph(graphs[2], pool=pool), streams.capture_origin():
                self._seg_c(static_x, labels_host)
            outs = self._parts
        with torch.no_grad():
            for t, sv in zip(state, saved):
                t.copy_(sv)
        self._graphs[key] = (graphs, static_x, outs)


def synthetic_waveform_batch(B, seconds, device, seed=1000, sr=22050):
    g = torch.Generator().manual_seed(seed)
    n = int(round(seconds * sr))
    t = torch.arange(n, dtype=torch.float32) / sr
    waves = []
    for i in range(B):
        f0 = 110.0 * 2 ** (torch.randint(0, 36, (1,), generator=g).item() / 12)
        y = torch.zeros(n)
        if i < B // 2:
            for h in range(1, 7):
                y += torch.exp(-3.0 * h * (t % 0.5)) * torch.sin(2 * torch.pi * f0 * h * t) / h
        else:
            for h in range(1, 9):
                y += torch.sin(2 * torch.pi * f0 * h * t + 0.3 * h * torch.sin(2 * torch.pi * 5.5 * t)) / h
        y += 0.01 * torch.randn(n, generator=g)
        waves.append(0.07 * y / y.pow(2).mean().sqrt())
    waves = torch.stack(waves).to(device)
    T = 1 + n // 256
    from .utilityFunctions import section_starts
    S = len(section_starts(T))
    x = torch.randn((B, S, 2, 287, 597), generator=g, dtype=torch.float32).to(device)
    mean = (0.01 * torch.randn(2, 513, generator=g)).to(device)
    std = (0.5 + torch.rand(2, 513, generator=g)).to(device)
    labels = torch.cat([torch.zeros(B // 2, dtype=torch.long), torch.ones(B - B // 2, dtype=torch.long)])
    return waves, x, mean, std, labels


def synthetic_batch(B, S, device, seed=1000):
    g = torch.Generator().manual_seed(seed)
    x = torch.randn((B, S, 2, 287, 597), generator=g, dtype=torch.float32)
    labels = torch.cat([torch.zeros(B // 2, dtype=torch.long), torch.ones(B - B // 2, dtype=torch.long)])
    return x.to(device), labels
```

audio-style-transfer_amd/csrc/skinny.hip:

```cpp
#include "ast_common.h"
#include "../../include/ast_hip.h"

namespace {

template <int NS, int NW = 4>
__global__ __launch_bounds__(64 * NW) void skinny_gemm_kernel(const float* __restrict__ x, const float* __restrict__ w,
                                                           const float* __restrict__ bias, float* __restrict__ y, int M, int N,
                                                           int K, int ldx, int ldw, int ldy, int relu,
                                                           const float* __restrict__ mul_mask, float* __restrict__ drop_mask,
                                                           float p, uint64_t seed, const int64_t* __restrict__ d_offset) {
  __shared__ f32x4 part[NW][64];
  const int lane = threadIdx.x & 63, wave = threadIdx.x >> 6;
  const int i = lane & 15, g = lane >> 4;
  const int n0 = blockIdx.x * 16, m0 = blockIdx.y * 16;
  constexpr int kslice = NS * 16;
  const int kb = wave * kslice;
  const bool nv = n0 + i < N, mv = m0 + i < M;
  const float* wr = w + (size_t)(nv ? n0 + i : 0) * ldw;
  const float* xr = x + (size_t)(mv ? m0 + i : 0) * ldx;
  f32x4 acc = {0.f, 0.f, 0.f, 0.f};
  float bq[4] = {0.f, 0.f, 0.f, 0.f};
  if (bias) {
#pragma unroll
    for (int q = 0; q < 4; ++q) { const int n = n0 + 4 * g + q; bq[q] = bias[n < N ? n : 0]; }
  }
  f32x4 wl[NS], xl[NS];
#pragma unroll
  for (int s = 0; s < NS; ++s) {
    const int k = kb + s * 16 + 4 * g;
    const bool kv = k < K;
    wl[s] = *reinterpret_cast<const f32x4*>(wr + (kv ? k : 0));
    xl[s] = *reinterpret_cast<const f32x4*>(xr + (kv ? k : 0));
  }
  __builtin_amdgcn_sched_barrier(0);
#pragma unroll
  for (int s = 0; s < NS; ++s) {
    const bool kv = kb + s * 16 + 4 * g < K;
    const f32x4 z = {0.f, 0.f, 0.f, 0.f};
    const f32x4 a = (kv && nv) ? wl[s] : z, b = (kv && mv) ? xl[s] : z;
#pragma unroll
    for (int e = 0; e < 4; ++e) acc = __builtin_amdgcn_mfma_f32_16x16x4f32(a[e], b[e], acc, 0, 0, 0);
  }
  part[wave][lane] = acc;
  __syncthreads();
  if (wave != 0) return;
  f32x4 r = part[0][lane];
#pragma unroll
  for (int q = 1; q < NW; ++q) { const f32x4 t = part[q][lane]; r[0] += t[0]; r[1] += t[1]; r[2] += t[2]; r[3] += t[3]; }
  const int m = m0 + i, nb = n0 + 4 * g;
  if (m >= M) return;
  const uint64_t base = drop_mask ? mix64(seed ^ mix64((uint64_t)(d_offset ? *d_offset : 0))) : 0;
  const float keep = 1.f / (1.f - p);
#pragma unroll
  for (int q = 0; q < 4; ++q) {
    const int n = nb + q;
    if (n < N) {
      const size_t o = (size_t)m * ldy + n;
      float v = r[q] + bq[q];
      if (relu) v = fmaxf(v, 0.f);
      if (drop_mask) {
        const float km = dropout_keep(base, o, p, keep);
        drop_mask[o] = (relu && v <= 0.f) ? 0.f : km;
        v *= km;
      }
      if (mul_mask) v *= mul_mask[o];
      y[o] = v;
    }
  }
}

template <int MS>
__global__ __launch_bounds__(256) void linear_wgrad_kernel(const float* __restrict__ dy, const float* __restrict__ x,
                                                            float* __restrict__ dW, float* __restrict__ db, int M, int N, int K,
                                                            int lddy, int ldw) {
  const int lane = threadIdx.x & 63, wave = threadIdx.x >> 6;
  const int i = lane & 15, g = lane >> 4;
  const int n0 = (blockIdx.y * 4 + wave) * 16, k0 = blockIdx.x * 64;
  if (n0 >= N) return;
  const bool nv = n0 + i < N;
  f32x4 acc[4];
#pragma unroll
  for (int t = 0; t < 4; ++t) acc[t] = f32x4{0.f, 0.f, 0.f, 0.f};
  float bsum = 0.f;
  float av[MS], bv[MS][4];
#pragma unroll
  for (int st = 0; st < MS; ++st) {
    const int m = st * 4 + g;
    const bool mv = m < M;
    av[st] = dy[(size_t)(mv ? m : 0) * lddy + (nv ? n0 + i : 0)];
#pragma unroll
    for (int t = 0; t < 4; ++t) {
      const int k = k0 + t * 16 + i;
      const bool kv = mv && k < K;
      bv[st][t] = x[(size_t)(kv ? m : 0) * K + (kv ? k : 0)];
    }
  }
  __builtin_amdgcn_sched_barrier(0);
#pragma unroll
  for (int st = 0; st < MS; ++st) {
    const bool mv = st * 4 + g < M;
    const float a = (mv && nv) ? av[st] : 0.f;
    bsum += a;
#pragma unroll
    for (int t = 0; t < 4; ++t) {
      const float b = (mv && k0 + t * 16 + i < K) ? bv[st][t] : 0.f;
      acc[t] = __builtin_amdgcn_mfma_f32_16x16x4f32(a, b, acc[t], 0, 0, 0);
    }
  }
  float old[4][4];
#pragma unroll
  for (int t = 0; t < 4; ++t) {
    const int k = k0 + t * 16 + i;
#pragma unroll
    for (int r = 0; r < 4; ++r) {
      const int n = n0 + 4 * g + r;
      old[t][r] = (k < K && n < N) ? dW[(size_t)n * ldw + k] : 0.f;
    }
  }
  __builtin_amdgcn_sched_barrier(0);
#pragma unroll
  for (int t = 0; t < 4; ++t) {
    const int k = k0 + t * 16 + i;
    if (k >= K) continue;
#pragma unroll
    for (int r = 0; r < 4; ++r) {
      const int n = n0 + 4 * g + r;
      if (n < N) dW[(size_t)n * ldw + k] = old[t][r] + acc[t][r];
    }
  }
  if (db && blockIdx.x == 0) {
    bsum += __shfl_xor(bsum, 16, 64);
    bsum += __shfl_xor(bsum, 32, 64);
    if (g == 0 && nv) db[n0 + i] += bsum;
  }
}
template <bool DET = false>
__global__ __launch_bounds__(256) void bigk_gemm_kernel(const float* __restrict__ x, const float* __restrict__ w,
                                                         const float* __restrict__ bias, float* __restrict__ y, int M, int N, int K,
                                                         int ldy) {
  __shared__ f32x4 part[4][64];
  const int lane = threadIdx.x & 63, wave = threadIdx.x >> 6;
  const int i = lane & 15, g = lane >> 4;
  const int n0 = blockIdx.x * 16, m0 = blockIdx.y * 16;
  const int kb = blockIdx.z * 1024 + wave * 256;
  const bool nv = n0 + i < N, mv = m0 + i < M;
  const float* wr = w + (size_t)(nv ? n0 + i : 0) * K;
  const float* xr = x + (size_t)(mv ? m0 + i : 0) * K;
  f32x4 acc = {0.f, 0.f, 0.f, 0.f};
#pragma unroll 1
  for (int sb = 0; sb < 32; sb += 8) {
    f32x2 wl[8], xl[8];
#pragma unroll
    for (int s = 0; s < 8; ++s) {
      const int k = kb + (sb + s) * 8 + 2 * g;
      const bool kv = k < K;
      wl[s] = *reinterpret_cast<const f32x2*>(wr + (kv ? k : 0));
      xl[s] = *reinterpret_cast<const f32x2*>(xr + (kv ? k : 0));
    }
    __builtin_amdgcn_sched_barrier(0);
#pragma unroll
    for (int s = 0; s < 8; ++s) {
      const bool kv = kb + (sb + s) * 8 + 2 * g < K;
      const f32x2 z = {0.f, 0.f};
      const f32x2 a = (kv && nv) ? wl[s] : z, b = (kv && mv) ? xl[s] : z;
#pragma unroll
      for (int e = 0; e < 2; ++e) acc = __builtin_amdgcn_mfma_f32_16x16x4f32(a[e], b[e], acc, 0, 0, 0);
    }
  }
  part[wave][lane] = acc;
  __syncthreads();
  if (wave != 0) return;
  f32x4 r = part[0][lane];
#pragma unroll
  for (int q = 1; q < 4; ++q) { const f32x4 t = part[q][lane]; r[0] += t[0]; r[1] += t[1]; r[2] += t[2]; r[3] += t[3]; }
  const int m = m0 + i, nb = n0 + 4 * g;
  if (m >= M) return;
#pragma unroll
  for (int q = 0; q < 4; ++q) {
    const int n = nb + q;
    if (n >= N) continue;
    const float v = r[q] + ((bias && blockIdx.z == 0) ? bias[n] : 0.f);
    if constexpr (DET) y[((size_t)blockIdx.z * M + m) * N + n] = v;
    else unsafeAtomicAdd(y + (size_t)m * ldy + n, v);
  }
}

template <bool DET = false>
__global__ __launch_bounds__(256) void bign_dgrad_kernel(const float* __restrict__ dy, const float* __restrict__ w,
                                                          float* __restrict__ dx, int M, int N, int K, int lddy) {
  const int lane = threadIdx.x & 63, wave = threadIdx.x >> 6;
  const int i = lane & 15, g = lane >> 4;
  const int nb0 = blockIdx.x * 512, m0 = blockIdx.y * 16;
  const int kt0 = wave * 4;
  const bool mv = m0 + i < M;
  const float* dr = dy + (size_t)(mv ? m0 + i : 0) * lddy;
  f32x4 acc[4];
#pragma unroll
  for (int t = 0; t < 4; ++t) acc[t] = f32x4{0.f, 0.f, 0.f, 0.f};
#pragma unroll 1
  for (int sb = 0; sb < 128; sb += 8) {
    float a[8][4], b[8];
#pragma unroll
    for (int s = 0; s < 8; ++s) {
      const int n = nb0 + (sb + s) * 4 + g;
      const bool nvv = n < N;
      b[s] = dr[nvv ? n : 0];
      const float* wrow = w + (size_t)(nvv ? n : 0) * K;
#pragma unroll
      for (int t = 0; t < 4; ++t) {
        const int k = (kt0 + t) * 16 + i;
        a[s][t] = wrow[k < K ? k : 0];
      }
    }
    __builtin_amdgcn_sched_barrier(0);
#pragma unroll
    for (int s = 0; s < 8; ++s) {
      const bool nvv = nb0 + (sb + s) * 4 + g < N;
      const float bq = (nvv && mv) ? b[s] : 0.f;
#pragma unroll
      for (int t = 0; t < 4; ++t) {
        const float aq = (nvv && (kt0 + t) * 16 + i < K) ? a[s][t] : 0.f;
        acc[t] = __builtin_amdgcn_mfma_f32_16x16x4f32(aq, bq, acc[t], 0, 0, 0);
      }
// ... 268 lines not shown
    for (int s = 0; s < 8; ++s) {
      const int k = kb + (sb + s) * 8 + 2 * g;
      const int kc = k < K ? k : 0;
      wl[s] = *reinterpret_cast<const f32x2*>(wr + kc);
#pragma unroll
      for (int t = 0; t < 4; ++t) xl[t][s] = *reinterpret_cast<const f32x2*>(xr[t] + kc);
    }
    __builtin_amdgcn_sched_barrier(0);
#pragma unroll
    for (int s = 0; s < 8; ++s) {
      const bool kv = kb + (sb + s) * 8 + 2 * g < K;
      const f32x2 z = {0.f, 0.f};
      const f32x2 a = (kv && nv) ? wl[s] : z;
#pragma unroll
      for (int t = 0; t < 4; ++t) {
        const f32x2 b = (kv && mv[t]) ? xl[t][s] : z;
#pragma unroll
        for (int e = 0; e < 2; ++e) acc[t] = __builtin_amdgcn_mfma_f32_16x16x4f32(a[e], b[e], acc[t], 0, 0, 0);
      }
    }
  }
#pragma unroll
  for (int t = 0; t < 4; ++t) part[wave][t][lane] = acc[t];
  __syncthreads();
  const int m = m0 + 16 * wave + i, nb = n0 + 4 * g;
  if (m >= M) return;
  f32x4 r = part[0][wave][lane];
#pragma unroll
  for (int q = 1; q < 4; ++q) { const f32x4 t = part[q][wave][lane]; r[0] += t[0]; r[1] += t[1]; r[2] += t[2]; r[3] += t[3]; }
#pragma unroll
  for (int q = 0; q < 4; ++q) {
    const int n = nb + q;
    if (n >= N) continue;
    const float v = r[q] + ((bias && blockIdx.z == 0) ? bias[n] : 0.f);
    if constexpr (DET) y[((size_t)blockIdx.z * M + m) * N + n] = v;
    else unsafeAtomicAdd(y + (size_t)m * ldy + n, v);
  }
}

template <bool DET = false>
__global__ __launch_bounds__(256) void bign_dgrad_wide_kernel(const float* __restrict__ dy, const float* __restrict__ w,
                                                               float* __restrict__ dx, int M, int N, int K, int lddy) {
  const int lane = threadIdx.x & 63, wave = threadIdx.x >> 6;
  const int i = lane & 15, g = lane >> 4;
  const int nb0 = blockIdx.x * 512, m0 = blockIdx.y * 64;
  const int kt0 = wave * 4;
  const float* dr[4];
  bool mv[4];
  f32x4 acc[4][4];
#pragma unroll
  for (int u = 0; u < 4; ++u) {
    const int m = m0 + 16 * u + i;
    mv[u] = m < M;
    dr[u] = dy + (size_t)(mv[u] ? m : 0) * lddy;
#pragma unroll
    for (int t = 0; t < 4; ++t) acc[u][t] = f32x4{0.f, 0.f, 0.f, 0.f};
  }
#pragma unroll 1
  for (int sb = 0; sb < 128; sb += 8) {
    float a[8][4], b[4][8];
#pragma unroll
    for (int s = 0; s < 8; ++s) {
      const int n = nb0 + (sb + s) * 4 + g;
      const int nc = n < N ? n : 0;
#pragma unroll
      for (int u = 0; u < 4; ++u) b[u][s] = dr[u][nc];
      const float* wrow = w + (size_t)nc * K;
#pragma unroll
      for (int t = 0; t < 4; ++t) {
        const int k = (kt0 + t) * 16 + i;
        a[s][t] = wrow[k < K ? k : 0];
      }
    }
    __builtin_amdgcn_sched_barrier(0);
#pragma unroll
    for (int s = 0; s < 8; ++s) {
      const bool nvv = nb0 + (sb + s) * 4 + g < N;
#pragma unroll
      for (int t = 0; t < 4; ++t) {
        const float aq = (nvv && (kt0 + t) * 16 + i < K) ? a[s][t] : 0.f;
#pragma unroll
        for (int u = 0; u < 4; ++u) {
          const float bq = (nvv && mv[u]) ? b[u][s] : 0.f;
          acc[u][t] = __builtin_amdgcn_mfma_f32_16x16x4f32(aq, bq, acc[u][t], 0, 0, 0);
        }
      }
    }
  }
#pragma unroll
  for (int u = 0; u < 4; ++u) {
    const int m = m0 + 16 * u + i;
    if (m >= M) continue;
#pragma unroll
    for (int t = 0; t < 4; ++t)
#pragma unroll
      for (int r = 0; r < 4; ++r) {
        const int k = (kt0 + t) * 16 + 4 * g + r;
        if (k >= K) continue;
        if constexpr (DET) dx[((size_t)blockIdx.x * M + m) * K + k] = acc[u][t][r];
        else unsafeAtomicAdd(dx + (size_t)m * K + k, acc[u][t][r]);
      }
  }
}
}

extern "C" int ast_linear_wgrad_batched_host(const void* host_table, int count, int max_tiles, void* stream) {
  if (!host_table || count <= 0 || max_tiles <= 0) AST_FAIL("ast_linear_wgrad_batched_host: bad args");
  const LinWg* recs = (const LinWg*)host_table;
  for (int c0 = 0; c0 < count; c0 += LINWG_MAX) {
    const int n = std::min(LINWG_MAX, count - c0);
    LinWgArgs args;
    memset(&args, 0, sizeof(args));
    memcpy(args.rec, recs + c0, sizeof(LinWg) * n);
    hipLaunchKernelGGL(linear_wgrad_batched_args_kernel, dim3(max_tiles, n), dim3(256), 0, (hipStream_t)stream, args);
  }
  AST_CHECK_LAUNCH();
  return 0;
}

extern "C" int ast_linear_wgrad_batched(const void* table, int count, int max_tiles, void* stream) {
  if (!table || count <= 0 || max_tiles <= 0) AST_FAIL("ast_linear_wgrad_batched: bad args");
  hipLaunchKernelGGL(linear_wgrad_batched_kernel, dim3(max_tiles, count), dim3(256), 0, (hipStream_t)stream, (const LinWg*)table);
  AST_CHECK_LAUNCH();
  return 0;
}

extern "C" int ast_skinny_gemm_ex(const float* x, const float* w, const float* bias, float* y, int M, int N, int K, int ldw, int ldy,
                                  int relu, const float* mul_mask, float* drop_mask, float p, uint64_t seed, const int64_t* d_offset,
                                  void* stream) {
  if (!x || !w || !y || M < 1 || M > 64 || N < 1 || K < 4 || (K & 3) || (ldw & 3)) AST_FAIL("ast_skinny_gemm: bad args M=%d N=%d K=%d", M, N, K);
  if ((((uintptr_t)x) | ((uintptr_t)w)) & 15) AST_FAIL("ast_skinny_gemm: operands must be 16-byte aligned");
  if (drop_mask && (p <= 0.f || p >= 1.f)) AST_FAIL("ast_skinny_gemm: dropout epilogue needs 0 < p < 1");
  const int steps = (K + 63) / 64;
  dim3 grid((N + 15) / 16, (M + 15) / 16);
  hipStream_t s = (hipStream_t)stream;
#define AST_SK(NS_) hipLaunchKernelGGL(skinny_gemm_kernel<NS_>, grid, dim3(256), 0, s, x, w, bias, y, M, N, K, K, ldw, ldy, relu, mul_mask, \
                                       drop_mask, p, seed, d_offset)
  if (steps <= 2) AST_SK(2);
  else if (steps <= 4) AST_SK(4);
  else if (steps <= 8) AST_SK(8);
  else if (steps <= 16) {
    hipLaunchKernelGGL((skinny_gemm_kernel<8, 8>), grid, dim3(512), 0, s, x, w, bias, y, M, N, K, K, ldw, ldy, relu, mul_mask, drop_mask, p,
                       seed, d_offset);
  }
  else AST_FAIL("ast_skinny_gemm: K=%d too large for the token path (<= 1024)", K);
#undef AST_SK
  AST_CHECK_LAUNCH();
  return 0;
}

extern "C" int ast_skinny_gemm(const float* x, const float* w, const float* bias, float* y, int M, int N, int K, int ldw, int ldy,
                               int relu, void* stream) {
  return ast_skinny_gemm_ex(x, w, bias, y, M, N, K, ldw, ldy, relu, nullptr, nullptr, 0.f, 0, nullptr, stream);
}

extern "C" int ast_linear_wgrad(const float* dy, const float* x, float* dW, float* db, int M, int N, int K, int lddy, int ldw,
                                void* stream) {
  if (!dy || !x || !dW || M < 1 || N < 1 || K < 1) AST_FAIL("ast_linear_wgrad: bad args");
  if (M > 64) AST_FAIL("ast_linear_wgrad: M=%d > 64 token rows", M);
  dim3 grid((K + 63) / 64, (N + 63) / 64);
  hipStream_t s = (hipStream_t)stream;
  if (M <= 16) hipLaunchKernelGGL(linear_wgrad_kernel<4>, grid, dim3(256), 0, s, dy, x, dW, db, M, N, K, lddy, ldw);
  else if (M <= 32) hipLaunchKernelGGL(linear_wgrad_kernel<8>, grid, dim3(256), 0, s, dy, x, dW, db, M, N, K, lddy, ldw);
  else hipLaunchKernelGGL(linear_wgrad_kernel<16>, grid, dim3(256), 0, s, dy, x, dW, db, M, N, K, lddy, ldw);
  AST_CHECK_LAUNCH();
  return 0;
}

extern "C" int ast_bigk_gemm(const float* x, const float* w, const float* bias, float* y, int M, int N, int K, int ldy, void* stream) {
  if (!x || !w || !y || M < 1 || M > 64 || N < 1 || K < 2 || (K & 1)) AST_FAIL("ast_bigk_gemm: bad args M=%d N=%d K=%d (K must be even)", M, N, K);
  if ((((uintptr_t)x) | ((uintptr_t)w)) & 7) AST_FAIL("ast_bigk_gemm: operands must be 8-byte aligned");
  dim3 grid((N + 15) / 16, (M + 15) / 16, (K + 1023) / 1024);
  AST_HIP(hipMemsetAsync(y, 0, sizeof(float) * (size_t)M * ldy, (hipStream_t)stream));
  hipLaunchKernelGGL(bigk_gemm_kernel<false>, grid, dim3(256), 0, (hipStream_t)stream, x, w, bias, y, M, N, K, ldy);
  AST_CHECK_LAUNCH();
  return 0;
}

extern "C" int ast_bign_dgrad(const float* dy, const float* w, float* dx, int M, int N, int K, int lddy, void* stream) {
  if (!dy || !w || !dx || M < 1 || M > 64 || N < 1 || K < 1 || K > 256) AST_FAIL("ast_bign_dgrad: bad args M=%d N=%d K=%d (K <= 256)", M, N, K);
  dim3 grid((N + 511) / 512, (M + 15) / 16);
  AST_HIP(hipMemsetAsync(dx, 0, sizeof(float) * (size_t)M * K, (hipStream_t)stream));
  hipLaunchKernelGGL(bign_dgrad_kernel<false>, grid, dim3(256), 0, (hipStream_t)stream, dy, w, dx, M, N, K, lddy);
  AST_CHECK_LAUNCH();
  return 0;
}

extern "C" int ast_ordered_sum(const float* parts, int64_t n, int nslots, int batches, float* out, int accumulate, void* stream);

extern "C" long ast_bigk_gemm_det_ws_floats(int M, int N, int K) {
  if (M < 1 || M > 64 || N < 1 || K < 2) return -1;
  return (long)((K + 1023) / 1024) * M * N;
}

extern "C" int ast_bigk_gemm_det(const float* x, const float* w, const float* bias, float* y, int M, int N, int K, float* ws, long ws_floats,
                                 void* stream) {
  if (!x || !w || !y || !ws || M < 1 || M > 64 || N < 1 || K < 2 || (K & 1)) AST_FAIL("ast_bigk_gemm_det: bad args M=%d N=%d K=%d (K must be even)", M, N, K);
  if ((((uintptr_t)x) | ((uintptr_t)w)) & 7) AST_FAIL("ast_bigk_gemm_det: operands must be 8-byte aligned");
  const int nz = (K + 1023) / 1024;
  if (nz > AST_DET_MAX_SLOTS || ws_floats < (long)nz * M * N) AST_FAIL("ast_bigk_gemm_det: ws needs %ld floats", (long)nz * M * N);
  dim3 grid((N + 15) / 16, (M + 15) / 16, nz);
  hipLaunchKernelGGL(bigk_gemm_kernel<true>, grid, dim3(256), 0, (hipStream_t)stream, x, w, bias, ws, M, N, K, N);
  AST_CHECK_LAUNCH();
  return ast_ordered_sum(ws, (int64_t)M * N, nz, 1, y, 0, stream);
}

extern "C" long ast_bign_dgrad_det_ws_floats(int M, int N, int K) {
  if (M < 1 || M > 64 || N < 1 || K < 1 || K > 256) return -1;
  return (long)((N + 511) / 512) * M * K;
}

extern "C" int ast_bign_dgrad_det(const float* dy, const float* w, float* dx, int M, int N, int K, int lddy, float* ws, long ws_floats,
                                  void* stream) {
  if (!dy || !w || !dx || !ws || M < 1 || M > 64 || N < 1 || K < 1 || K > 256) AST_FAIL("ast_bign_dgrad_det: bad args M=%d N=%d K=%d (K <= 256)", M, N, K);
  const int nx = (N + 511) / 512;
  if (nx > AST_DET_MAX_SLOTS || ws_floats < (long)nx * M * K) AST_FAIL("ast_bign_dgrad_det: ws needs %ld floats", (long)nx * M * K);
  dim3 grid(nx, (M + 15) / 16);
  hipLaunchKernelGGL(bign_dgrad_kernel<true>, grid, dim3(256), 0, (hipStream_t)stream, dy, w, ws, M, N, K, lddy);
  AST_CHECK_LAUNCH();
  return ast_ordered_sum(ws, (int64_t)M * K, nx, 1, dx, 0, stream);
}

#define AST_WIDE_ROWS_OK(M) ((M) > 64 && (M) <= AST_WIDE_MAX_ROWS)

extern "C" int ast_skinny_gemm_wide_ex(const float* x, const float* w, const float* bias, float* y, int M, int N, int K, int ldw, int ldy,
                                       int relu, const float* mul_mask, float* drop_mask, float p, uint64_t seed, const int64_t* d_offset,
                                       void* stream) {
  if (!x || !w || !y || !AST_WIDE_ROWS_OK(M) || N < 1 || K < 4 || (K & 3) || (ldw & 3) || ldw < K || ldy < N)
    AST_FAIL("ast_skinny_gemm_wide: bad args M=%d (65..%d) N=%d K=%d ldw=%d ldy=%d", M, AST_WIDE_MAX_ROWS, N, K, ldw, ldy);
  if ((((uintptr_t)x) | ((uintptr_t)w)) & 15) AST_FAIL("ast_skinny_gemm_wide: operands must be 16-byte aligned");
  if (drop_mask && (p <= 0.f || p >= 1.f)) AST_FAIL("ast_skinny_gemm_wide: dropout epilogue needs 0 < p < 1");
  const int steps = (K + 63) / 64;
  if (steps > 16) AST_FAIL("ast_skinny_gemm_wide: K=%d too large for the token path (<= 1024)", K);
  dim3 grid((N + 15) / 16, (M + 63) / 64);
  hipStream_t s = (hipStream_t)stream;
#define AST_SKW(NS_, NW_) hipLaunchKernelGGL((skinny_gemm_wide_kernel<NS_, NW_>), grid, dim3(64 * NW_), 0, s, x, w, bias, y, M, N, K, K, ldw, \
                                             ldy, relu, mul_mask, drop_mask, p, seed, d_offset)
  if (steps <= 2) AST_SKW(2, 4);
  else if (steps <= 4) AST_SKW(4, 4);
  else if (steps <= 8) AST_SKW(8, 4);
  else AST_SKW(8, 8);
#undef AST_SKW
  AST_CHECK_LAUNCH();
  return 0;
}

extern "C" int ast_skinny_gemm_wide(const float* x, const float* w, const float* bias, float* y, int M, int N, int K, int ldw, int ldy,
                                    int relu, void* stream) {
  return ast_skinny_gemm_wide_ex(x, w, bias, y, M, N, K, ldw, ldy, relu, nullptr, nullptr, 0.f, 0, nullptr, stream);
}

extern "C" int ast_linear_wgrad_wide(const float* dy, const float* x, float* dW, float* db, int M, int N, int K, int lddy, int ldw,
                                     void* stream) {
  if (!dy || !x || !dW || !AST_WIDE_ROWS_OK(M) || N < 1 || K < 1 || lddy < N || ldw < K)
    AST_FAIL("ast_linear_wgrad_wide: bad args M=%d (65..%d) N=%d K=%d lddy=%d ldw=%d", M, AST_WIDE_MAX_ROWS, N, K, lddy, ldw);
  dim3 grid((K + 63) / 64, (N + 63) / 64);
  if (grid.y > 65535) AST_FAIL("ast_linear_wgrad_wide: N=%d too large", N);
  hipLaunchKernelGGL(linear_wgrad_wide_kernel, grid, dim3(256), 0, (hipStream_t)stream, dy, x, dW, db, M, N, K, lddy, ldw);
  AST_CHECK_LAUNCH();
  return 0;
}

extern "C" int ast_bigk_gemm_wide(const float* x, const float* w, const float* bias, float* y, int M, int N, int K, int ldy, void* stream) {
  if (!x || !w || !y || !AST_WIDE_ROWS_OK(M) || N < 1 || K < 2 || (K & 1) || ldy < N)
    AST_FAIL("ast_bigk_gemm_wide: bad args M=%d (65..%d) N=%d K=%d (K must be even) ldy=%d", M, AST_WIDE_MAX_ROWS, N, K, ldy);
  if ((((uintptr_t)x) | ((uintptr_t)w)) & 7) AST_FAIL("ast_bigk_gemm_wide: operands must be 8-byte aligned");
  const int nz = (K + 1023) / 1024;
  if (nz > 65535) AST_FAIL("ast_bigk_gemm_wide: K=%d too large", K);
  dim3 grid((N + 15) / 16, (M + 63) / 64, nz);
  AST_HIP(hipMemsetAsync(y, 0, sizeof(float) * (size_t)M * ldy, (hipStream_t)stream));
  hipLaunchKernelGGL(bigk_gemm_wide_kernel<false>, grid, dim3(256), 0, (hipStream_t)stream, x, w, bias, y, M, N, K, ldy);
  AST_CHECK_LAUNCH();
  return 0;
}

extern "C" long ast_bigk_gemm_wide_det_ws_floats(int M, int N, int K) {
  if (!AST_WIDE_ROWS_OK(M) || N < 1 || K < 2 || (K & 1) || (K + 1023) / 1024 > 65535) return -1;
  return (long)((K + 1023) / 1024) * M * N;
}

extern "C" int ast_bigk_gemm_wide_det(const float* x, const float* w, const float* bias, float* y, int M, int N, int K, float* ws,
                                      long ws_floats, void* stream) {
  if (!x || !w || !y || !ws || !AST_WIDE_ROWS_OK(M) || N < 1 || K < 2 || (K & 1))
    AST_FAIL("ast_bigk_gemm_wide_det: bad args M=%d (65..%d) N=%d K=%d (K must be even)", M, AST_WIDE_MAX_ROWS, N, K);
  if ((((uintptr_t)x) | ((uintptr_t)w)) & 7) AST_FAIL("ast_bigk_gemm_wide_det: operands must be 8-byte aligned");
  const int nz = (K + 1023) / 1024;
  if (nz > 65535 || ws_floats < (long)nz * M * N) AST_FAIL("ast_bigk_gemm_wide_det: ws needs %ld floats", (long)nz * M * N);
  dim3 grid((N + 15) / 16, (M + 63) / 64, nz);
  hipLaunchKernelGGL(bigk_gemm_wide_kernel<true>, grid, dim3(256), 0, (hipStream_t)stream, x, w, bias, ws, M, N, K, N);
  AST_CHECK_LAUNCH();
  return ast_ordered_sum(ws, (int64_t)M * N, nz, 1, y, 0, stream);
}

extern "C" int ast_bign_dgrad_wide(const float* dy, const float* w, float* dx, int M, int N, int K, int lddy, void* stream) {
  if (!dy || !w || !dx || !AST_WIDE_ROWS_OK(M) || N < 1 || K < 1 || K > 256 || lddy < N)
    AST_FAIL("ast_bign_dgrad_wide: bad args M=%d (65..%d) N=%d K=%d (K <= 256) lddy=%d", M, AST_WIDE_MAX_ROWS, N, K, lddy);
  dim3 grid((N + 511) / 512, (M + 63) / 64);
  AST_HIP(hipMemsetAsync(dx, 0, sizeof(float) * (size_t)M * K, (hipStream_t)stream));
  hipLaunchKernelGGL(bign_dgrad_wide_kernel<false>, grid, dim3(256), 0, (hipStream_t)stream, dy, w, dx, M, N, K, lddy);
  AST_CHECK_LAUNCH();
  return 0;
}

extern "C" long ast_bign_dgrad_wide_det_ws_floats(int M, int N, int K) {
  if (!AST_WIDE_ROWS_OK(M) || N < 1 || K < 1 || K > 256 || (N + 511) / 512 > AST_DET_MAX_SLOTS) return -1;
  return (long)((N + 511) / 512) * M * K;
// ... 14 lines not shown
```

include/ast_hip.h:

```cpp
#ifndef AST_HIP_H
#define AST_HIP_H
#include <stddef.h>
#include <stdint.h>
#ifdef __cplusplus
extern "C" {
#endif

#define AST_DTYPE_F32 0
#define AST_DTYPE_BF16 1
#define AST_MAX_TAPS 9

int ast_version(void);
const char* ast_last_error(void);

typedef struct ast_gather_t {
  int32_t N, Hs, Ws, Cs;
  int32_t Hm, Wm;
  int32_t sh, sw, oh, ow;
  int32_t Hd, Wd, Cd;
  int32_t dsh, dsw, doh, dow;
  int32_t ntaps, wtaps;
  int32_t tap[AST_MAX_TAPS];
} ast_gather_t;

int ast_igemm(const void* src, const void* wgt, const float* bias, void* dst,
              const ast_gather_t* g, int dtype, int flags, float* ws, long ws_floats, void* stream);
int ast_igemm_bn(const void* src, const void* wgt, const float* bias, void* dst, const ast_gather_t* g, int dtype, int flags,
                 float* ws, long ws_floats, const void* bn_x, const float* bn_scale, const float* bn_shift, void* stream);
long ast_igemm_ws_floats(const ast_gather_t* g, int dtype);
int ast_igemm_plan(const ast_gather_t* g, int dtype, int* out5);
int ast_pconv_variant(const ast_gather_t* g, int dtype, int* out4);

int ast_wgrad(const void* dy, const void* src, float* dw, const ast_gather_t* g,
              int dtype, void* stream);
int ast_wgrad_rep(const void* dy, const void* src, float* dw, const ast_gather_t* g, int dtype, int nrep, void* stream);
#define AST_MAX_SLAB_RECS 48
int ast_wgrad_slab(const void* dy, const void* src, float* slabs, const ast_gather_t* g, int dtype, int nslabs, int* slices_out,
                   void* stream);
int ast_slab_sum(float* const* bases, const int64_t* floats_per_copy, const int* slabs, int nrec, void* stream);

int ast_skinny_gemm(const float* x, const float* w, const float* bias, float* y, int M, int N, int K, int ldw,
                    int ldy, int relu, void* stream);
int ast_skinny_gemm_ex(const float* x, const float* w, const float* bias, float* y, int M, int N, int K, int ldw, int ldy,
                       int relu, const float* mul_mask, float* drop_mask, float p, uint64_t seed, const int64_t* d_offset,
                       void* stream);
int ast_bigk_gemm(const float* x, const float* w, const float* bias, float* y, int M, int N, int K, int ldy, void* stream);
int ast_bign_dgrad(const float* dy, const float* w, float* dx, int M, int N, int K, int lddy, void* stream);
int ast_linear_wgrad(const float* dy, const float* x, float* dW, float* db, int M, int N, int K, int lddy, int ldw,
                     void* stream);

int ast_linear_wgrad_batched(const void* table, int count, int max_tiles, void* stream);
int ast_linear_wgrad_batched_host(const void* host_table, int count, int max_tiles, void* stream);

int ast_nchw_to_nhwc(const float* x, void* y, int N, int C, int H, int W, int64_t sn, int64_t sc,
                     int64_t sh, int Cp, int dtype, void* stream);
int ast_nhwc_to_nchw(const void* x, float* y, int N, int C, int H, int W, int Cp, int dtype, void* stream);
int ast_cast(const void* x, int dtype_in, void* y, int dtype_out, int64_t n, void* stream);

typedef struct ast_weight_desc_t {
  const float* w;
  float* u;
  float* v;
  float* sigma;
  float* scratch;
  void* wf;
  void* wb;
  int32_t Co, Ci, KK, s_co, s_ci, Cop, Cip;
  int32_t power_iter;
  float* dwp;
  float* grad;
  float* inner;
  int32_t dwp_from_wb;
  int32_t dwp_replicas;
} ast_weight_desc_t;
long ast_sn_scratch_floats(int Co, int ncols);
int ast_weights_prepare_t(const ast_weight_desc_t* descs, const int* dtypes, int n, int max_co, int max_cols,
                          const void* tiles, int ntiles, void* stream);
int ast_weight_grads_flush_t(const ast_weight_desc_t* descs, const void* tiles, int ntiles, void* stream);
int ast_weight_grad_unpack(const float* dwp, int from_wb, const float* w, const float* u, const float* v,
                           const float* sigma, float* g_orig, int Co, int Ci, int KK, int s_co, int s_ci,
                           int Cop, int Cip, float* scratch, void* stream);

int ast_chan_stats(const void* x, float* sums, int N, int HW, int C, int dtype, int assume_zeroed, void* stream);
int ast_norm_finalize(float* sums, int zero_sums, int64_t* num_batches_tracked ,
                      int N, int HW, int C, int Creal, int instance,
                      const float* gamma, const float* beta, float* running_mean, float* running_var,
                      int eval_mode, float eps, float* mean, float* rstd, float* scale, float* shift,
                      long count, void* stream);
int ast_affine_act(const void* x, const float* scale, const float* shift, const void* r,
                   const float* scale2, const float* shift2, void* y, int N, int HW, int C,
                   int flags, int dtype, void* stream);
int ast_bn_apply_fwd(const void* x, const void* r, void* y, const float* tab1, int rows1, long count1, const float* tab2,
                     const float* gamma1, const float* beta1, float* running_mean, float* running_var, int64_t* num_batches_tracked,
                     float eps1, const float* gamma2, const float* beta2, float eps2, float* out1, float* out2, int N, int HW, int C,
                     int Creal, int flags , int dtype, void* stream);
int ast_bn_apply_bwd(const void* dy, const void* x, const void* r, void* dx, void* dr, const float* tab3, int rows, long count,
                     const float* gamma1, const float* mean1, const float* rstd1, float* dgamma1, float* dbeta1,
                     const float* gamma2, const float* mean2, const float* rstd2, float* dgamma2, float* dbeta2,
                     const float* scale1, const float* shift1, const float* scale2, const float* shift2, int N, int HW, int C,
                     int Creal, int flags, int dtype, void* stream);
int ast_norm_bwd_sums(const void* dy, const void* y, const void* x, const void* r, float* sums3,
                      int N, int HW, int C, int relu, int dtype, int assume_zeroed, void* stream);
int ast_norm_bwd_finalize(float* sums3, int zero_sums, int N, int HW, int C, int Creal,
                          const float* gamma1, const float* mean1, const float* rstd1,
                          float* dgamma1, float* dbeta1, float* k1,
                          const float* gamma2, const float* mean2, const float* rstd2,
                          float* dgamma2, float* dbeta2, float* k2, void* stream);
int ast_norm_bwd_finalize_n(float* sums3, int zero_sums, int N, int HW, int C, int Creal, const float* gamma1,
                            const float* mean1, const float* rstd1, float* dgamma1, float* dbeta1, float* k1,
                            const float* gamma2, const float* mean2, const float* rstd2, float* dgamma2,
                            float* dbeta2, float* k2, long count, void* stream);
int ast_norm_bwd_apply(const void* dy, const void* y, const void* x, const void* r,
                       const float* k1, const float* k2, void* dx, void* dr,
                       int N, int HW, int C, int relu, int dtype, void* stream);
int ast_norm_bwd_sums_pre(const void* dy, const void* y, const void* x, const void* r, float* sums3, int N, int HW,
                          int C, int relu, int dtype, int assume_zeroed, const float* scale1, const float* shift1,
                          const float* scale2, const float* shift2, void* stream);
int ast_norm_bwd_apply_pre(const void* dy, const void* y, const void* x, const void* r, const float* k1,
                           const float* k2, void* dx, void* dr, int N, int HW, int C, int relu, int dtype,
                           const float* scale1, const float* shift1, const float* scale2, const float* shift2,
                           void* stream);

int ast_layernorm_fwd(const void* x, const float* gamma, const float* beta, void* y, float* mean,
                      float* rstd, int rows, int D, float eps, int dtype, void* stream);
int ast_layernorm_bwd(const void* dy, const void* x, const float* gamma, const float* mean,
                      const float* rstd, void* dx, float* dgamma, float* dbeta, int rows, int D,
                      int dtype, void* stream);

int ast_add_drop_ln_fwd(const float* x, const float* sub, float* mask, float* s_out, const float* gamma, const float* beta,
                        float* y, float* mean, float* rstd, int rows, int D, float eps, float p, uint64_t seed,
                        const int64_t* d_offset, void* stream);
int ast_add_drop_ln_bwd(const float* dy, const float* ds_ext, const float* s, const float* gamma, const float* mean,
                        const float* rstd, const float* mask, float* dx, float* dsub, float* dgamma, float* dbeta, int rows,
                        int D, void* stream);

int ast_rowmix(const float* A, const float* X, float* Y, int R_out, int R_in, int D, void* stream);

int ast_adaptive_pool_fwd(const void* x, void* y, int N, int H, int W, int C, int Ho, int Wo, int dtype, void* stream);
int ast_adaptive_pool_bwd(const void* dy, void* dx, int N, int H, int W, int C, int Ho, int Wo, int dtype, void* stream);
int ast_bilinear_fwd(const void* x, float* y, int N, int C, int Cp, int H, int W, int Ho, int Wo, int dtype, void* stream);
int ast_bilinear_bwd(const float* dy, void* dx, int N, int C, int Cp, int H, int W, int Ho, int Wo, int dtype, void* stream);

#define AST_ATTN_MAX_L 1024
int ast_attn_fwd(const float* q, const float* k, const float* v, float* o, float* probs,
                 int B, int H, int Lq, int Lk, int dh, int ldq, int ldk, int ldo, int causal,
                 const float* drop_mask, void* stream);
int ast_attn_bwd(const float* dout, const float* q, const float* k, const float* v, const float* probs,
                 float* dq, float* dk, float* dv, int B, int H, int Lq, int Lk, int dh, int ldq,
                 int ldk, int ldo, const float* drop_mask, void* stream);
int ast_attn_fwd_p(const float* q, const float* k, const float* v, float* o, float* probs, int B, int H, int Lq, int Lk,
                   int dh, int ldq, int ldk, int ldo, int causal, const float* drop_mask, float p, uint64_t seed,
                   const int64_t* d_offset, void* stream);
int ast_attn_bwd_p(const float* dout, const float* q, const float* k, const float* v, const float* probs, float* dq, float* dk,
                   float* dv, int B, int H, int Lq, int Lk, int dh, int ldq, int ldk, int ldo, const float* drop_mask,
                   float p, uint64_t seed, const int64_t* d_offset, void* stream);

int ast_colsum_acc(const void* x, int64_t rows, int C, int Creal, float* out, int dtype, void* stream);
int ast_add(const void* a, const void* b, void* y, int64_t n, int dtype, void* stream);
int ast_relu_bwd(const void* dy, const void* y, void* dx, int64_t n, int dtype, void* stream);
int ast_dropout_fwd(const float* x, float* y, float* mask, int64_t n, float p, uint64_t seed, const int64_t* d_offset, void* stream);
int ast_dropout_mask(float* mask, int64_t n, float p, uint64_t seed, const int64_t* d_offset, void* stream);
int ast_mul(const void* a, const float* mask, void* y, int64_t n, int dtype, void* stream);

int ast_recon_loss(const float* out, const float* tgt, int64_t tgt_ld, int B, int S, int T, int Fq,
                   float w_mse, float w_mag, float w_phase, float w_temporal, float w_spectral,
                   float* sums, float* grad, void* stream);
#define AST_RECON_SLOTS 64
int ast_recon_loss_total(const float* out, const float* tgt, int64_t tgt_ld, int B, int S, int T, int Fq, const float* coef5,
                         const float* inv5, float* ws, float* res11, float* grad, void* stream);
int ast_infonce(const float* emb, const int32_t* labels, int B, int D, float temperature,
                float* loss, float* demb, float* ws , void* stream);
int ast_margin(const float* cls, int C, int D, float margin, float* loss, float* dcls, void* stream);
int ast_hsic(const float* s, const float* c, int B, int D, float* loss, float* ds, float* dc,
             float* ws , void* stream);
int ast_crosscov(const float* s, const float* c, int B, int D, float* loss, float* ds, float* dc, float* ws, void* stream);
int ast_cross_entropy(const float* logits, const int32_t* target, int R, int C, float* loss, float* dlogits, void* stream);
int ast_softmax_entropy(const float* logits, int R, int C, float* loss, float* dlogits, void* stream);

int ast_scale(const float* x, const float* dscale, float hscale, float* y, int64_t n, int accumulate, void* stream);

int ast_counter_incr(int64_t* c, void* stream);
int ast_sumsq(const float* x, int64_t n, float* out , void* stream);
int ast_adam(float* p, const float* g, float* m, float* v, int64_t n, float lr, float b1, float b2,
             float eps, float wd, const int64_t* d_step, const float* gnorm_sq, float max_norm, void* stream);

#define AST_MAX_STEP_SCALARS 16
int ast_adam_dev(float* p, const float* g, float* m, float* v, int64_t n, const float* d_hyper , float b1, float b2,
                 float eps, float wd, const int64_t* d_step, const float* gnorm_sq, void* stream);
int ast_set_values(float* dst, const float* host_vals, int n, void* stream);
int ast_weighted_sum(const float* const* terms, const int* widx, int n, const float* weights, float* out, void* stream);
int ast_weighted_sum_bwd(const float* g, const int* widx, int n, const float* weights, float* grads, void* stream);

int ast_istft(const float* spec, int Bc, int T, float* frames_ws, float* wave, void* stream);
int ast_bin_stats_acc(const float* x, float* mean_acc, float* var_acc, int C, int T, int F, void* stream);
int ast_zscore(const float* x, const float* mean, const float* std_, float* out, int C, int T, int F, float eps, void* stream);
int ast_sections_overlap_avg(const float* sections, float* out, int Bc, int S, int wind, int hop, int F_in, int F_out,
                             int out_T, void* stream);
int ast_stft_sections(const float* wave, int Bc, int nsamp, const float* mean, const float* std_,
// ... 68 lines not shown
```

Before: 5304 audio-seconds/sec.

## Fuse residual-add/dropout/LayerNorm prologue into following skinny token GEMM

Adds a deferred-launch mechanism (PendingRows/_Prologue) so the residual add, dropout and LayerNorm before a token linear or FFN are recorded rather than launched. A new HIP kernel, skinny_gemm_ln, recomputes the normalisation per workgroup and feeds the result straight into the MFMA GEMM; block column 0 writes the normalised rows and statistics for autograd. The aim is to remove separate kernel launches and a round trip through global memory for the small transformer token tensors. In exchange, every GEMM workgroup repeats the LayerNorm arithmetic, and the encoder and decoder layer control flow becomes more complex.

```diff
diff --git a/audio-style-transfer_amd/ast_amd/_lib.py b/audio-style-transfer_amd/ast_amd/_lib.py
--- a/audio-style-transfer_amd/ast_amd/_lib.py
+++ b/audio-style-transfer_amd/ast_amd/_lib.py
@@ -38,6 +38,8 @@
     "ast_wgrad": ([vp, vp, vp, C.POINTER(Gather), i32, vp], i32),
     "ast_skinny_gemm": ([vp, vp, vp, vp, i32, i32, i32, i32, i32, i32, vp], i32),
     "ast_skinny_gemm_ex": ([vp, vp, vp, vp, i32, i32, i32, i32, i32, i32, vp, vp, f32, C.c_uint64, vp, vp], i32),
+    "ast_skinny_gemm_ln": ([vp, vp, vp, vp, vp, vp, vp, vp, vp, f32, f32, C.c_uint64, vp,
+                            vp, vp, vp, i32, i32, i32, i32, i32, i32, vp, f32, C.c_uint64, vp, vp], i32),
     "ast_bigk_gemm": ([vp, vp, vp, vp, i32, i32, i32, i32, vp], i32),
     "ast_bign_dgrad": ([vp, vp, vp, i32, i32, i32, i32, vp], i32),
     "ast_linear_wgrad": ([vp, vp, vp, vp, i32, i32, i32, i32, i32, vp], i32),
diff --git a/audio-style-transfer_amd/ast_amd/config.py b/audio-style-transfer_amd/ast_amd/config.py
--- a/audio-style-transfer_amd/ast_amd/config.py
+++ b/audio-style-transfer_amd/ast_amd/config.py
@@ -13,6 +13,7 @@
 import os as _os
 fused_tokens = _os.environ.get("AST_FUSED_TOKENS", "1") != "0"
 tok_programs = int(_os.environ.get("AST_TOK_PROGRAMS", "0"))
+tok_prologue = _os.environ.get("AST_TOK_PROLOGUE", "1") != "0"
 
 fused_bn_stats = _os.environ.get("AST_FUSED_BN_STATS", "1") != "0"
 
diff --git a/audio-style-transfer_amd/ast_amd/content_encoder.py b/audio-style-transfer_amd/ast_amd/content_encoder.py
--- a/audio-style-transfer_amd/ast_amd/content_encoder.py
+++ b/audio-style-transfer_amd/ast_amd/content_encoder.py
@@ -39,10 +39,9 @@
         feat = L.linear(feat, self._proj)
         if self._inp is not None:
             feat = L.linear(feat, self._inp)
-        seq = L.layer_norm(self.pos_encoder(feat.view(B, S, -1)), self.norm)
+        seq = L.layer_norm(self.pos_encoder(feat.view(B, S, -1)), self.norm, pending=config.tok_programs == 0)
         if config.tok_programs > 0 and tokprog.encoder_stack_ok(seq, self._layers):
             seq = tokprog.encoder_stack(seq, self._layers, self.training, xcd=1)
         else:
-            for lyr in self._layers:
-                seq = lyr(seq, self.training)
+            seq = ops.rows_of(L.run_stack(self._layers, seq, self.training))
         return seq
diff --git a/audio-style-transfer_amd/ast_amd/layers.py b/audio-style-transfer_amd/ast_amd/layers.py
--- a/audio-style-transfer_amd/ast_amd/layers.py
+++ b/audio-style-transfer_amd/ast_amd/layers.py
@@ -424,8 +424,21 @@
     return _bn_apply(y, bn, training, relu, stats)
 
 
-def layer_norm(x, ln: nn.LayerNorm):
+def layer_norm(x, ln: nn.LayerNorm, pending=False):
+    if pending:
+        return ops.layer_norm_pending(ops.rows_of(x), ln)
     return ops.LayerNormFn.apply(x, ln.weight, ln.bias, ln.eps)
+
+
+def norm_linear(x, ln: nn.LayerNorm, pw):
+    pn = x.norm(ln) if isinstance(x, ops.PendingRows) else ops.layer_norm_pending(x, ln)
+    return pn.linear(pw)
+
+
+def run_stack(layers, x, *args):
+    for lyr in layers:
+        x = lyr(x, *args, pending_out=True)
+    return x
 
 
 class MHA:
@@ -443,14 +456,15 @@
     def __call__(self, x, mem, training, p_drop, causal=False):
         B, Lq, d = x.shape
         dh = d // self.h
+        proj = x.linear if isinstance(x, ops.PendingRows) else (lambda pw: linear(x.reshape(B * Lq, d), pw))
         if self.cross:
             Lk = mem.shape[1]
-            q = linear(x.reshape(B * Lq, d), self.q)
+            q = proj(self.q)
             kv = linear(mem.reshape(B * Lk, d), self.kv)
             k_off, v_off = 0, d
         else:
             Lk = Lq
-            q = kv = linear(x.reshape(B * Lq, d), self.qkv)
+            q = kv = proj(self.qkv)
             k_off, v_off = d, 2 * d
         o = ops.AttnCoreFn.apply(q, kv, B, self.h, Lq, Lk, dh, k_off, v_off, causal, float(p_drop) if training else 0.0)
         return linear(o, self.out).view(B, Lq, d)
@@ -464,9 +478,16 @@
         self.ff1 = bank.add(layer.linear1.weight, "linear", tok_dtype, bias=layer.linear1.bias)
         self.ff2 = bank.add(layer.linear2.weight, "linear", tok_dtype, bias=layer.linear2.bias)
 
-    def __call__(self, x, training):
+    def __call__(self, x, training, pending_out=False):
         l, p = self.l, self.l.dropout.p
         B, L, d = x.shape
+        if config.fused_tokens and config.tok_prologue:
+            a = self.attn(x, None, training, l.self_attn.dropout)
+            pn = ops.add_drop_ln_pending(ops.rows_of(x), a, l.norm1, l.dropout1.p, training)
+            h = pn.ffn(self.ff1, self.ff2, p, training)
+            out = ops.add_drop_ln_pending(pn.value, h.view(B, L, d), l.norm2, l.dropout2.p, training)
+            return out if pending_out else out.value
+        x = ops.rows_of(x)
         if not config.fused_tokens:
             x = layer_norm(x + ops.dropout(self.attn(x, None, training, l.self_attn.dropout), l.dropout1.p, training), l.norm1)
             h = ops.dropout(linear(x.reshape(B * L, d), self.ff1, relu=True), p, training)
@@ -487,9 +508,19 @@
         self.ff1 = bank.add(layer.linear1.weight, "linear", tok_dtype, bias=layer.linear1.bias)
         self.ff2 = bank.add(layer.linear2.weight, "linear", tok_dtype, bias=layer.linear2.bias)
 
-    def __call__(self, x, memory, training):
+    def __call__(self, x, memory, training, pending_out=False):
         l = self.l
         B, L, d = x.shape
+        if config.fused_tokens and config.tok_prologue:
+            pn = x.norm(l.norm1) if isinstance(x, ops.PendingRows) else ops.layer_norm_pending(x, l.norm1)
+            a = self.sa(pn, None, training, l.self_attn.dropout, causal=True)
+            pn = ops.add_drop_ln_pending(pn.s, a, l.norm2, l.dropout1.p, training)
+            a = self.ca(pn, memory, training, l.multihead_attn.dropout)
+            pn = ops.add_drop_ln_pending(pn.s, a, l.norm3, l.dropout2.p, training)
+            h = pn.ffn(self.ff1, self.ff2, l.dropout.p, training)
+            out = ops.add_drop_ln_pending(pn.s, h.view(B, L, d), None, l.dropout3.p, training)
+            return out if pending_out else out.s
+        x = ops.rows_of(x)
         if not config.fused_tokens:
             h = layer_norm(x, l.norm1)
             x = x + ops.dropout(self.sa(h, None, training, l.self_attn.dropout, causal=True), l.dropout1.p, training)
diff --git a/audio-style-transfer_amd/ast_amd/new_decoder.py b/audio-style-transfer_amd/ast_amd/new_decoder.py
--- a/audio-style-transfer_amd/ast_amd/new_decoder.py
+++ b/audio-style-transfer_amd/ast_amd/new_decoder.py
@@ -90,7 +90,7 @@
     def _generate(self, tok):
         B, S, D = tok.shape
         tr = self.training
-        h = L.linear(L.layer_norm(tok, self.output_norm).reshape(B * S, D), self._s2f)
+        h = L.norm_linear(tok, self.output_norm, self._s2f)
         h = ops.CastFn.apply(h, L.img_dtype()).view(B * S, self.F_compressed, self.T_compressed, 1)
         h = torch.cat([h, h.new_zeros(B * S, self.F_compressed, self.T_compressed, 7)], dim=3)
         for pw, i in zip(self._dec[:4], (0, 3, 6, 9)):
@@ -119,12 +119,11 @@
         self._prepare()
         return self._memory(content_emb, class_emb)
 
-    def _stack(self, tgt, memory):
+    def _stack(self, tgt, memory, pending=False):
         if config.tok_programs > 0 and tokprog.decoder_stack_ok(tgt, memory, self._layers):
             return tokprog.decoder_stack(tgt, memory, self._layers, self.training)
-        for lyr in self._layers:
-            tgt = lyr(tgt, memory, self.training)
-        return tgt
+        tgt = L.run_stack(self._layers, tgt, memory, self.training)
+        return tgt if pending else ops.rows_of(tgt)
 
     def encode_target(self, y):
         self._prepare()
@@ -138,7 +137,7 @@
             emb = self._encode_nhwc(ops.nchw_to_nhwc(y.view(B * S, *y.shape[2:]), L.img_dtype())).view(B, S, self.d_model)
         tgt = torch.cat([self.start_token.expand(B, 1, -1), emb[:, :-1, :]], dim=1)
         tgt = L.layer_norm(self.pos_encoding(tgt), self.input_norm)
-        return self._generate(self._stack(tgt, memory))
+        return self._generate(self._stack(tgt, memory, pending=True))
 
     def forward_training(self, y, memory):
         self._prepare()
diff --git a/audio-style-transfer_amd/ast_amd/ops.py b/audio-style-transfer_amd/ast_amd/ops.py
--- a/audio-style-transfer_amd/ast_amd/ops.py
+++ b/audio-style-transfer_amd/ast_amd/ops.py
@@ -430,6 +430,147 @@
     return rows <= SKINNY_MAX_ROWS or (config.deterministic and rows <= WIDE_MAX_ROWS)
 
 
+class _Prologue:
+    defer = None
+    absorb = None
+
+    def __init__(self):
+        self.add = self.norm = None
+        self.done = False
+
+    @classmethod
+    def take(cls, slot):
+        rec = getattr(cls, slot)
+        setattr(cls, slot, None)
+        return rec
+
+    def launch(self):
+        if self.done:
+            return
+        self.done = True
+        if self.add is not None:
+            x2, sub2, mask, s, ln, y, mean, rstd, rows, p, seed = self.add
+            check(lib().ast_add_drop_ln_fwd(ptr(x2), ptr(sub2), ptr(mask), ptr(s), ptr(ln.weight) if ln is not None else None,
+                                            ptr(ln.bias) if ln is not None else None, ptr(y), ptr(mean), ptr(rstd), rows, s.shape[1],
+                                            float(ln.eps) if ln is not None else 0.0, float(p), seed,
+                                            ptr(_DropState.counter) if p > 0.0 else None, stream()), "ast_add_drop_ln_fwd")
+        if self.norm is not None:
+            x2, gamma, beta, y, mean, rstd, rows, eps = self.norm
+            check(lib().ast_layernorm_fwd(ptr(x2), ptr(gamma), ptr(beta), ptr(y), ptr(mean), ptr(rstd), rows, x2.shape[1], eps,
+                                          dcode(x2.dtype), stream()), "ast_layernorm_fwd")
+
+    def absorbable(self, pw, rows):
+        if self.done or rows > SKINNY_MAX_ROWS or not (pw.KK == 1 and pw.u is None and pw.Ci == pw.Cip == 256):
+            return False
+        if self.add is not None and self.add[4] is None and self.norm is None:
+            return False
+        return (pw.weight.data_ptr() + 4 * pw.w_off) % 16 == 0 and pw.s_co % 4 == 0
+
+    def launch_fused(self, w, b, y, N, ldw, ldy, relu, drop_mask=None, p=0.0, seed=0, ctr=None):
+        assert not self.done
+        self.done = True
+        x2 = sub2 = mask = s = gamma = beta = h = mean = rstd = None
+        rows, eps, p_in, seed_in = 0, 0.0, 0.0, 0
+        if self.add is not None:
+            x2, sub2, mask, s, ln, h, mean, rstd, rows, p_in, seed_in = self.add
+            if ln is not None:
+                gamma, beta, eps = ln.weight, ln.bias, float(ln.eps)
+        if self.norm is not None:
+            xn, gamma, beta, h, mean, rstd, rows, eps = self.norm
+            if self.add is None:
+                x2 = xn
+        check(lib().ast_skinny_gemm_ln(ptr(x2), ptr(sub2), ptr(mask), ptr(s), ptr(gamma), ptr(beta), ptr(h), ptr(mean), ptr(rstd), eps,
+                                       float(p_in), seed_in, ptr(_DropState.counter) if p_in > 0.0 else None, w, b, ptr(y), rows, N, 256,
+                                       ldw, ldy, int(relu), ptr(drop_mask), float(p), seed, ptr(ctr), stream()), "ast_skinny_gemm_ln")
+
+
+def _prologue_ok(t):
+    return (config.tok_prologue and config.fused_tokens and config.tok_programs == 0 and not config.deterministic and t.is_cuda and t.dtype == torch.float32
+            and t.dim() >= 2 and t.shape[-1] == 256 and 0 < t.numel() <= 256 * SKINNY_MAX_ROWS and t.is_contiguous()
+            and t.data_ptr() % 16 == 0)
+
+
+class PendingRows:
+
+    def __init__(self, rec, s, h):
+        self._rec, self._s, self._h = rec, s, h
+        self.shape = s.shape
+
+    def _ready(self):
+        if self._rec is not None:
+            self._rec.launch()
+            self._rec = None
+
+    @property
+    def s(self):
+        self._ready()
+        return self._s
+
+    @property
+    def value(self):
+        self._ready()
+        return self._h if self._h is not None else self._s
+
+    def _consume(self, pws, apply):
+        rec = self._rec
+        rows = self._s.numel() // self.shape[-1]
+        rows2d = (self._h if self._h is not None else self._s).reshape(rows, self.shape[-1])
+        if rec is None or not all(_skinny_ok(pw, rows) for pw in pws) or not rec.absorbable(pws[0], rows):
+            self._ready()
+            return apply(rows2d)
+        _Prologue.absorb = rec
+        try:
+            return apply(rows2d)
+        finally:
+            _Prologue.absorb = None
+            self._ready()
+
+    def linear(self, pw, relu=False):
+        y = self._consume((pw,), lambda r: LinearFn.apply(r, pw.weight, pw, relu))
+        return y if pw.Cop == pw.Co else y[:, :pw.Co]
+
+    def ffn(self, pw1, pw2, p, training):
+        return self._consume((pw1, pw2), lambda r: ffn(r, pw1, pw2, p, training))
+
+    def norm(self, ln):
+        rec = self._rec
+        if rec is None or rec.done or self._h is not None or rec.norm is not None:
+            return layer_norm_pending(self.value, ln)
+        _Prologue.defer = rec
+        try:
+            h = LayerNormFn.apply(self._s, ln.weight, ln.bias, ln.eps)
+        finally:
+            _Prologue.defer = None
+        self._rec = None
+        return PendingRows(rec, self._s, h)
+
+
+def rows_of(x):
+    return x.value if isinstance(x, PendingRows) else x
+
+
+def layer_norm_pending(x, ln):
+    rec = None
+    if _prologue_ok(x):
+        rec = _Prologue.defer = _Prologue()
+    try:
+        h = LayerNormFn.apply(x, ln.weight, ln.bias, ln.eps)
+    finally:
+        _Prologue.defer = None
+    return PendingRows(rec, x, h)
+
+
+def add_drop_ln_pending(x, sub, ln, p, training):
+    rec = None
+    if _prologue_ok(sub) and (x is None or _prologue_ok(x)):
+        rec = _Prologue.defer = _Prologue()
+    try:
+        out = AddDropLNFn.apply(x, sub, ln, float(p) if training else 0.0)
+    finally:
+        _Prologue.defer = None
+    return PendingRows(rec, out, None) if ln is None else PendingRows(rec, out[0], out[1])
+
+
 class LinearFn(torch.autograd.Function):
 
     @staticmethod
@@ -440,11 +581,18 @@
         ctx.skinny = (_token_rows_ok(rows) and pw.KK == 1 and pw.u is None and pw.Ci == pw.Cip
                       and (rows <= SKINNY_MAX_ROWS or x.dtype == torch.float32))
         y = torch.empty((rows, pw.Cop), dtype=x.dtype, device=x.device)
+        rec = _Prologue.take("absorb")
+        if rec is not None and not (ctx.skinny and rec.absorbable(pw, rows)):
+            rec.launch()
+            rec = None
         if ctx.skinny:
             if pw.Cop != pw.Co:
                 y.zero_()
             b = None if pw.bias is None else pw.bias.data_ptr() + 4 * pw.b_off
-            _skinny_gemm(rows, ptr(x), pw.weight.data_ptr() + 4 * pw.w_off, b, ptr(y), pw.Co, pw.Ci, pw.s_co, pw.Cop, int(relu))
+            if rec is not None:
+                rec.launch_fused(pw.weight.data_ptr() + 4 * pw.w_off, b, y, pw.Co, pw.s_co, pw.Cop, relu)
+            else:
+                _skinny_gemm(rows, ptr(x), pw.weight.data_ptr() + 4 * pw.w_off, b, ptr(y), pw.Co, pw.Ci, pw.s_co, pw.Cop, int(relu))
         else:
             g, _ = gather_direct(rows, 1, 1, pw.Cip, pw.Cop, 1, 1, 0)
             _igemm(x, pw.wf, pw.bias_ptr_tensor(), y, g, 2 if relu else 0)
@@ -552,8 +700,16 @@
             _DropState.calls += 1
             seed, ctr = _DropState.seed + 7919 * _DropState.calls, _DropState.counter
             mask = torch.empty_like(h)
-        _skinny_gemm_ex(rows, ptr(x), pw1.weight.data_ptr() + 4 * pw1.w_off, pw1.bias.data_ptr() + 4 * pw1.b_off, ptr(h),
-                        pw1.Co, pw1.Ci, pw1.s_co, pw1.Cop, 1, None, ptr(mask), float(p), seed, ptr(ctr))
+        rec = _Prologue.take("absorb")
+        if rec is not None and not rec.absorbable(pw1, rows):
+            rec.launch()
+            rec = None
+        if rec is not None:
+            rec.launch_fused(pw1.weight.data_ptr() + 4 * pw1.w_off, pw1.bias.data_ptr() + 4 * pw1.b_off, h, pw1.Co, pw1.s_co, pw1.Cop, 1,
+                             mask, float(p), seed, ctr)
+        else:
+            _skinny_gemm_ex(rows, ptr(x), pw1.weight.data_ptr() + 4 * pw1.w_off, pw1.bias.data_ptr() + 4 * pw1.b_off, ptr(h),
+                            pw1.Co, pw1.Ci, pw1.s_co, pw1.Cop, 1, None, ptr(mask), float(p), seed, ptr(ctr))
         _skinny_gemm(rows, ptr(h), pw2.weight.data_ptr() + 4 * pw2.w_off, pw2.bias.data_ptr() + 4 * pw2.b_off, ptr(y),
                      pw2.Co, pw2.Ci, pw2.s_co, pw2.Cop, 0)
         ctx.save_for_backward(x, h, mask)
@@ -850,8 +1006,12 @@
         y = torch.empty_like(x2)
         mean = torch.empty(rows, dtype=torch.float32, device=x.device)
         rstd = torch.empty_like(mean)
-        check(lib().ast_layernorm_fwd(ptr(x2), ptr(gamma), ptr(beta), ptr(y), ptr(mean), ptr(rstd), rows, D, eps,
-                                      dcode(x2.dtype), stream()), "ast_layernorm_fwd")
+        rec = _Prologue.take("defer")
+        if rec is not None:
+            rec.norm = (x2, gamma, beta, y, mean, rstd, rows, float(eps))
+        else:
+            check(lib().ast_layernorm_fwd(ptr(x2), ptr(gamma), ptr(beta), ptr(y), ptr(mean), ptr(rstd), rows, D, eps,
+                                          dcode(x2.dtype), stream()), "ast_layernorm_fwd")
         ctx.save_for_backward(x2, mean, rstd)
         ctx.gamma, ctx.beta, ctx.shape = gamma, beta, shape
         return y.view(shape)
@@ -896,10 +1056,14 @@
             y = torch.empty_like(sub2)
             mean = torch.empty(rows, dtype=torch.float32, device=sub.device)
             rstd = torch.empty_like(mean)
-        check(lib().ast_add_drop_ln_fwd(ptr(x2), ptr(sub2), ptr(mask), ptr(s), ptr(ln.weight) if ln is not None else None,
-                                        ptr(ln.bias) if ln is not None else None, ptr(y), ptr(mean), ptr(rstd), rows, D,
-                                        float(ln.eps) if ln is not None else 0.0, float(p), seed,
-                                        ptr(_DropState.counter) if p > 0.0 else None, stream()), "ast_add_drop_ln_fwd")
+        rec = _Prologue.take("defer")
+        if rec is not None:
+            rec.add = (x2, sub2, mask, s, ln, y, mean, rstd, rows, float(p), seed)
+        else:
+            check(lib().ast_add_drop_ln_fwd(ptr(x2), ptr(sub2), ptr(mask), ptr(s), ptr(ln.weight) if ln is not None else None,
+                                            ptr(ln.bias) if ln is not None else None, ptr(y), ptr(mean), ptr(rstd), rows, D,
+                                            float(ln.eps) if ln is not None else 0.0, float(p), seed,
+                                            ptr(_DropState.counter) if p > 0.0 else None, stream()), "ast_add_drop_ln_fwd")
         ctx.save_for_backward(s, mean, rstd, mask)
         ctx.ln, ctx.shape, ctx.has_x = ln, shape, x is not None
         if ln is None:
diff --git a/audio-style-transfer_amd/ast_amd/style_encoder.py b/audio-style-transfer_amd/ast_amd/style_encoder.py
--- a/audio-style-transfer_amd/ast_amd/style_encoder.py
+++ b/audio-style-transfer_amd/ast_amd/style_encoder.py
@@ -144,12 +144,11 @@
         seq = feat.view(B, S, -1)
         if self.use_cls:
             seq = torch.cat([self.cls_token.expand(B, -1, -1), seq], dim=1)
-        seq = L.layer_norm(self.pos_encoder(seq), self.norm)
+        seq = L.layer_norm(self.pos_encoder(seq), self.norm, pending=config.tok_programs == 0)
         if config.tok_programs > 0 and tokprog.encoder_stack_ok(seq, self._layers):
             seq = tokprog.encoder_stack(seq, self._layers, self.training, xcd=0)
         else:
-            for lyr in self._layers:
-                seq = lyr(seq, self.training)
+            seq = ops.rows_of(L.run_stack(self._layers, seq, self.training))
         style_emb = seq[:, 0, :] if self.use_cls else seq.mean(dim=1)
         class_emb = class_prototypes(style_emb, labels) if labels is not None else None
         return style_emb, class_emb
diff --git a/audio-style-transfer_amd/ast_amd/train.py b/audio-style-transfer_amd/ast_amd/train.py
--- a/audio-style-transfer_amd/ast_amd/train.py
+++ b/audio-style-transfer_amd/ast_amd/train.py
@@ -659,7 +659,7 @@
         c = self.cfg
         fe = tuple(t.data_ptr() for t in (self._frontend or ())) + tuple(t.data_ptr() for t in (self._frontend_cqt or ()))
         return (tuple(x.shape), tuple(labels_host.tolist()), config.compute_dtype, c.use_nce, c.use_hsic, c.use_adv, segmented,
-                tuple(c.betas), c.eps, c.max_grad_norm > 0, fe, self._deterministic())
+                tuple(c.betas), c.eps, c.max_grad_norm > 0, fe, self._deterministic(), config.tok_prologue)
 
     def _mutable_state(self):
         ts = [self.G.flat_p, self.G.m, self.G.v, self.G.step, self.D.flat_p, self.D.m, self.D.v, self.D.step]
diff --git a/audio-style-transfer_amd/csrc/skinny.hip b/audio-style-transfer_amd/csrc/skinny.hip
--- a/audio-style-transfer_amd/csrc/skinny.hip
+++ b/audio-style-transfer_amd/csrc/skinny.hip
@@ -69,6 +69,131 @@
   }
 }
 
+__global__ __launch_bounds__(256) void skinny_gemm_ln_kernel(const float* __restrict__ x, const float* __restrict__ sub,
+                                                             float* __restrict__ mask, float* __restrict__ s_out,
+                                                             const float* __restrict__ gamma, const float* __restrict__ beta,
+                                                             float* __restrict__ h_out, float* __restrict__ mean, float* __restrict__ rstd,
+                                                             float eps, float p_in, uint64_t seed_in, const int64_t* __restrict__ d_offset_in,
+                                                             const float* __restrict__ w, const float* __restrict__ bias, float* __restrict__ y,
+                                                             int M, int N, int ldw, int ldy, int relu, float* __restrict__ drop_mask, float p,
+                                                             uint64_t seed, const int64_t* __restrict__ d_offset) {
+  constexpr int D = 256, NS = 4, NW = 4;
+  __shared__ f32x4 part[NW][64];
+  __shared__ float red[2][NW][16];
+  const int lane = threadIdx.x & 63, wave = threadIdx.x >> 6;
+  const int i = lane & 15, g = lane >> 4;
+  const int n0 = blockIdx.x * 16, m0 = blockIdx.y * 16;
+  const int kb = wave * (NS * 16);
+  const bool nv = n0 + i < N, mv = m0 + i < M;
+  const float* wr = w + (size_t)(nv ? n0 + i : 0) * ldw;
+  const size_t ro = (size_t)(mv ? m0 + i : 0) * D;
+  f32x4 acc = {0.f, 0.f, 0.f, 0.f};
+  float bq[4] = {0.f, 0.f, 0.f, 0.f};
+  if (bias) {
+#pragma unroll
+    for (int q = 0; q < 4; ++q) { const int n = n0 + 4 * g + q; bq[q] = bias[n < N ? n : 0]; }
+  }
+  const f32x4 z = {0.f, 0.f, 0.f, 0.f};
+  f32x4 wl[NS], xl[NS], sl[NS], gl[NS], bl[NS];
+#pragma unroll
+  for (int s = 0; s < NS; ++s) {
+    const int k = kb + s * 16 + 4 * g;
+    wl[s] = *reinterpret_cast<const f32x4*>(wr + k);
+    xl[s] = x ? *reinterpret_cast<const f32x4*>(x + ro + k) : z;
+    sl[s] = sub ? *reinterpret_cast<const f32x4*>(sub + ro + k) : z;
+    gl[s] = gamma ? *reinterpret_cast<const f32x4*>(gamma + k) : z;
+    bl[s] = gamma ? *reinterpret_cast<const f32x4*>(beta + k) : z;
+  }
+  const bool drop_in = sub && p_in > 0.f;
+  const uint64_t base_in = drop_in ? mix64(seed_in ^ mix64((uint64_t)(d_offset_in ? *d_offset_in : 0))) : 0;
+  __builtin_amdgcn_sched_barrier(0);
+  const bool st = blockIdx.x == 0 && mv;
+  const float keep_in = 1.f / (1.f - p_in);
+  f32x4 v[NS];
+#pragma unroll
+  for (int s = 0; s < NS; ++s) {
+    const size_t o = ro + kb + s * 16 + 4 * g;
+    if (sub) {
+      f32x4 sv2 = sl[s];
+      if (drop_in) {
+        f32x4 m4;
+#pragma unroll
+        for (int e = 0; e < 4; ++e) { m4[e] = dropout_keep(base_in, o + e, p_in, keep_in); sv2[e] *= m4[e]; }
+        if (st) *reinterpret_cast<f32x4*>(mask + o) = m4;
+      }
+#pragma unroll
+      for (int e = 0; e < 4; ++e) v[s][e] = x ? sv2[e] + xl[s][e] : sv2[e];
+      if (st) *reinterpret_cast<f32x4*>(s_out + o) = v[s];
+    } else {
+      v[s] = xl[s];
+    }
+  }
+  if (gamma) {
+    float t[NS];
+#pragma unroll
+    for (int s = 0; s < NS; ++s) {
+      t[s] = v[s][0] + v[s][1] + v[s][2] + v[s][3];
+      t[s] += __shfl_xor(t[s], 16, 64);
+      t[s] += __shfl_xor(t[s], 32, 64);
+    }
+    if (g == 0) red[0][wave][i] = (t[0] + t[3]) + (t[2] + t[1]);
+    __syncthreads();
+    const float m = ((red[0][0][i] + red[0][1][i]) + (red[0][2][i] + red[0][3][i])) / D;
+#pragma unroll
+    for (int s = 0; s < NS; ++s) {
+      float q = 0.f;
+#pragma unroll
+      for (int e = 0; e < 4; ++e) { const float d = v[s][e] - m; q += d * d; }
+      q += __shfl_xor(q, 16, 64);
+      q += __shfl_xor(q, 32, 64);
+      t[s] = q;
+    }
+    if (g == 0) red[1][wave][i] = (t[0] + t[3]) + (t[2] + t[1]);
+    __syncthreads();
+    const float r = rsqrtf(((red[1][0][i] + red[1][1][i]) + (red[1][2][i] + red[1][3][i])) / D + eps);
+#pragma unroll
+    for (int s = 0; s < NS; ++s) {
+      f32x4 y4;
+#pragma unroll
+      for (int e = 0; e < 4; ++e) y4[e] = (v[s][e] - m) * r * gl[s][e] + bl[s][e];
+      v[s] = y4;
+      if (st) *reinterpret_cast<f32x4*>(h_out + ro + kb + s * 16 + 4 * g) = y4;
+    }
+    if (st && wave == 0 && g == 0) { mean[m0 + i] = m; rstd[m0 + i] = r; }
+  }
+#pragma unroll
+  for (int s = 0; s < NS; ++s) {
+    const f32x4 a = nv ? wl[s] : z, b = mv ? v[s] : z;
+#pragma unroll
+    for (int e = 0; e < 4; ++e) acc = __builtin_amdgcn_mfma_f32_16x16x4f32(a[e], b[e], acc, 0, 0, 0);
+  }
+  part[wave][lane] = acc;
+  __syncthreads();
+  if (wave != 0) return;
+  f32x4 r4 = part[0][lane];
+#pragma unroll
+  for (int q = 1; q < NW; ++q) { const f32x4 t4 = part[q][lane]; r4[0] += t4[0]; r4[1] += t4[1]; r4[2] += t4[2]; r4[3] += t4[3]; }
+  const int m = m0 + i, nb = n0 + 4 * g;
+  if (m >= M) return;
+  const uint64_t base = drop_mask ? mix64(seed ^ mix64((uint64_t)(d_offset ? *d_offset : 0))) : 0;
+  const float keep = 1.f / (1.f - p);
+#pragma unroll
+  for (int q = 0; q < 4; ++q) {
+    const int n = nb + q;
+    if (n < N) {
+      const size_t o = (size_t)m * ldy + n;
+      float val = r4[q] + bq[q];
+      if (relu) val = fmaxf(val, 0.f);
+      if (drop_mask) {
+        const float km = dropout_keep(base, o, p, keep);
+        drop_mask[o] = (relu && val <= 0.f) ? 0.f : km;
+        val *= km;
+      }
+      y[o] = val;
+    }
+  }
+}
+
 template <int MS>
 __global__ __launch_bounds__(256) void linear_wgrad_kernel(const float* __restrict__ dy, const float* __restrict__ x,
                                                             float* __restrict__ dW, float* __restrict__ db, int M, int N, int K,
@@ -643,6 +768,28 @@
 extern "C" int ast_skinny_gemm(const float* x, const float* w, const float* bias, float* y, int M, int N, int K, int ldw, int ldy,
                                int relu, void* stream) {
   return ast_skinny_gemm_ex(x, w, bias, y, M, N, K, ldw, ldy, relu, nullptr, nullptr, 0.f, 0, nullptr, stream);
+}
+
+extern "C" int ast_skinny_gemm_ln(const float* x, const float* sub, float* mask, float* s_out, const float* gamma, const float* beta,
+                                  float* h_out, float* mean, float* rstd, float eps, float p_in, uint64_t seed_in, const int64_t* d_offset_in,
+                                  const float* w, const float* bias, float* y, int M, int N, int K, int ldw, int ldy, int relu,
+                                  float* drop_mask, float p, uint64_t seed, const int64_t* d_offset, void* stream) {
+  if (!w || !y || M < 1 || M > 64 || N < 1 || (ldw & 3) || ldw < K || ldy < N) AST_FAIL("ast_skinny_gemm_ln: bad args M=%d (<= 64) N=%d ldw=%d ldy=%d", M, N, ldw, ldy);
+  if (K != 256) AST_FAIL("ast_skinny_gemm_ln: K=%d; a workgroup holds whole rows only at K == 256 (the LayerNorm width)", K);
+  if (!x && !sub) AST_FAIL("ast_skinny_gemm_ln: no input");
+  if (!sub && !gamma) AST_FAIL("ast_skinny_gemm_ln: neither a residual term nor a LayerNorm: use ast_skinny_gemm");
+  if (sub && !s_out) AST_FAIL("ast_skinny_gemm_ln: the residual sum needs s_out");
+  if (p_in < 0.f || p_in >= 1.f || (p_in > 0.f && (!sub || !mask))) AST_FAIL("ast_skinny_gemm_ln: dropout needs 0 <= p < 1, sub and a mask buffer");
+  if (gamma && (!beta || !h_out || !mean || !rstd)) AST_FAIL("ast_skinny_gemm_ln: LayerNorm outputs missing");
+  if ((((uintptr_t)x) | ((uintptr_t)sub) | ((uintptr_t)mask) | ((uintptr_t)s_out) | ((uintptr_t)gamma) | ((uintptr_t)beta) | ((uintptr_t)h_out) |
+       ((uintptr_t)w)) & 15)
+    AST_FAIL("ast_skinny_gemm_ln: operands must be 16-byte aligned");
+  if (drop_mask && (p <= 0.f || p >= 1.f)) AST_FAIL("ast_skinny_gemm_ln: dropout epilogue needs 0 < p < 1");
+  dim3 grid((N + 15) / 16, (M + 15) / 16);
+  hipLaunchKernelGGL(skinny_gemm_ln_kernel, grid, dim3(256), 0, (hipStream_t)stream, x, sub, mask, s_out, gamma, beta, h_out, mean, rstd, eps, p_in,
+                     seed_in, d_offset_in, w, bias, y, M, N, ldw, ldy, relu, drop_mask, p, seed, d_offset);
+  AST_CHECK_LAUNCH();
+  return 0;
 }
 
 extern "C" int ast_linear_wgrad(const float* dy, const float* x, float* dW, float* db, int M, int N, int K, int lddy, int ldw,
diff --git a/include/ast_hip.h b/include/ast_hip.h
--- a/include/ast_hip.h
+++ b/include/ast_hip.h
@@ -44,6 +44,10 @@
 int ast_skinny_gemm_ex(const float* x, const float* w, const float* bias, float* y, int M, int N, int K, int ldw, int ldy,
                        int relu, const float* mul_mask, float* drop_mask, float p, uint64_t seed, const int64_t* d_offset,
                        void* stream);
+int ast_skinny_gemm_ln(const float* x, const float* sub, float* mask, float* s_out, const float* gamma, const float* beta, float* h_out,
+                       float* mean, float* rstd, float eps, float p_in, uint64_t seed_in, const int64_t* d_offset_in, const float* w,
+                       const float* bias, float* y, int M, int N, int K, int ldw, int ldy, int relu, float* drop_mask, float p,
+                       uint64_t seed, const int64_t* d_offset, void* stream);
 int ast_bigk_gemm(const float* x, const float* w, const float* bias, float* y, int M, int N, int K, int ldy, void* stream);
 int ast_bign_dgrad(const float* dy, const float* w, float* dx, int M, int N, int K, int lddy, void* stream);
 int ast_linear_wgrad(const float* dy, const float* x, float* dW, float* db, int M, int N, int K, int lddy, int ldw,
```

New measurement: 5346 audio-seconds/sec (median of 6 runs). Within noise of the previous version (+0.8%).
